# fanagislab/DBG_assembly

Hardware: AMD Instinct MI355X
Metric: M k-mers/s hashed (k=31, 150 bp) (higher is better)
Workload: dtype u64

## Files before the change

### dbg_assembly_amd/csrc/dbgk_host_level1.h

```cpp
#pragma once

#include "dbgk_l1_form.h"

constexpr L1Limits kL1Limits{(uint32_t)kL1Threads, (uint32_t)kPkWords, kPrefixMaxW, kPrefixPipeMaxB, (uint32_t)kWL1Threads, kWPkWords, kWPipePkWords};
static_assert(DBGK_L1_THREADS != 1024 || DBGK_L1_MAXB != 1024 || kL1Limits == L1Limits{}, "dbgk_l1_form.h: the defaults of L1Limits are the product build's geometry");

template <class Fn>
struct L1Row {
	L1Form form;
	Fn fn;
	uint32_t lds;
};
template <int DBG, int WIDE_D, int C, bool RAGGED, bool LIN, bool... REST>
constexpr uint32_t uniform_lds() { return LIN ? sizeof(UniformLdsLin<LIN ? C : 8>) : sizeof(UniformLds); }
#define DBGK_ROW(...) {l1_uniform(__VA_ARGS__), &k_extract_scatter_uniform<__VA_ARGS__>, uniform_lds<__VA_ARGS__>()},
static const L1Row<decltype(&k_extract_scatter_uniform<>)> kL1UniformRows[] = {DBGK_L1_UNIFORM_ROWS(DBGK_ROW)};
#undef DBGK_ROW
#define DBGK_ROW(...) {l1_prefix(__VA_ARGS__), &k_extract_scatter_prefix<__VA_ARGS__>, sizeof(PrefixLds)},
static const L1Row<decltype(&k_extract_scatter_prefix<>)> kL1PrefixRows[] = {DBGK_L1_PREFIX_ROWS(DBGK_ROW)};
#undef DBGK_ROW
#define DBGK_ROW(...) {l1_flat(__VA_ARGS__), &k_extract_scatter<__VA_ARGS__>, sizeof(ScatterLds)},
static const L1Row<decltype(&k_extract_scatter<false>)> kL1FlatRows[] = {DBGK_L1_FLAT_ROWS(DBGK_ROW)};
#undef DBGK_ROW
#define DBGK_ROW(...) {l1_flat_lin(__VA_ARGS__), &k_extract_scatter_lin<__VA_ARGS__>, sizeof(ScatterLdsLin<8>)},
static const L1Row<decltype(&k_extract_scatter_lin<false>)> kL1FlatLinRows[] = {DBGK_L1_FLAT_LIN_ROWS(DBGK_ROW)};
#undef DBGK_ROW
#define DBGK_ROW(...) {l1_wide_flat(__VA_ARGS__), &k_wide_scatter_l1<__VA_ARGS__>, sizeof(WL1Lds)},
static const L1Row<decltype(&k_wide_scatter_l1<false, 0>)> kL1WideFlatRows[] = {DBGK_L1_WIDE_FLAT_ROWS(DBGK_ROW)};
#undef DBGK_ROW
#define DBGK_ROW(WD, PIPE) {l1_wide_uniform(WD, PIPE), &k_wide_scatter_l1_uniform<WD, PIPE>, PIPE ? sizeof(WL1PipeLds) : sizeof(WL1Lds)},
static const L1Row<decltype(&k_wide_scatter_l1_uniform<0>)> kL1WideUniformRows[] = {DBGK_L1_WIDE_UNIFORM_ROWS(DBGK_ROW)};
#undef DBGK_ROW

template <class Fn, size_t N>
static int l1_set_lds_attrs(const L1Row<Fn> (&rows)[N])
{
	for (const L1Row<Fn> &r : rows)
		HIPCHK(hipFuncSetAttribute(reinterpret_cast<const void *>(r.fn), hipFuncAttributeMaxDynamicSharedMemorySize, (int)r.lds));
	return DBGK_OK;
}
static int l1_register_lds(bool wide)
{
	int rc;
	if (wide) return (rc = l1_set_lds_attrs(kL1WideFlatRows)) ? rc : l1_set_lds_attrs(kL1WideUniformRows);
	if ((rc = l1_set_lds_attrs(kL1UniformRows)) || (rc = l1_set_lds_attrs(kL1PrefixRows)) || (rc = l1_set_lds_attrs(kL1FlatRows))) return rc;
	return l1_set_lds_attrs(kL1FlatLinRows);
}

template <class Fn, size_t N, class... Args>
static int l1_launch(const L1Row<Fn> (&rows)[N], const L1Form &form, uint64_t grid, int threads, hipStream_t stream, Args... args)
{
	for (const L1Row<Fn> &r : rows)
		if (r.form == form) {
			hipLaunchKernelGGL(r.fn, dim3((uint32_t)grid), dim3(threads), r.lds, stream, args...);
			return DBGK_OK;
		}
	char text[192];
	l1_form_text(form, text, sizeof text);
	g_last_error = std::string("no level-1 kernel for the form ") + text;
	return DBGK_ERR_ARG;
}

static L1Facts l1_facts(const dbgk_handle *h, bool wrec)
{
	L1Facts f;
	f.lim = kL1Limits;
	f.part = h->part; f.seed = h->seed; f.kfreq = h->kfreq; f.wide = h->wide; f.wrec = wrec;
	f.kmer_size = h->cfg.kmer_size;
	f.max_read_len = (uint64_t)h->cfg.max_read_len;
	f.n1 = h->geom.n1; f.kf = h->geom.kf; f.geom_size = h->geom.size; f.size = h->size;
	auto hook_int = [](const char *name) { const char *v = dbgk_hook(name); return v ? atoi(v) : -1; };
	f.l1_linear = hook_int("l1_linear");
	f.l1_prefix = hook_int("l1_prefix");
	f.l1_plain = dbgk_hook("l1_plain") != nullptr;
	f.wide_l1_plain = dbgk_hook("wide_l1_plain") != nullptr;
	f.l1_flat = DBGK_EXPERIMENT_ENV("DBGK_L1_FLAT") != nullptr;
	const char *dbg = DBGK_EXPERIMENT_ENV("DBGK_DEBUG_MODE"), *lin_c = DBGK_EXPERIMENT_ENV("DBGK_L1_LINEAR_C");
	f.dbg_set = dbg != nullptr;
	f.dbg_mode = dbg ? atoi(dbg) : 0;
	f.no_reg = DBGK_EXPERIMENT_ENV("DBGK_L1_NO_REG") != nullptr;
	f.lin_c = lin_c ? (atoi(lin_c) == 12 ? 12 : 8) : 0;
	return f;
}

static int ensure_prefix_scratch(dbgk_handle *h, uint64_t n_reads, uint64_t n_bases, bool need_packed)
{
	const uint64_t tiles = (n_bases / 15 + n_reads) / kL1Threads + 2;
	if (n_reads > h->pf_cap_reads || tiles > h->pf_cap_tiles) {
		HIPCHK(hipStreamSynchronize(h->stream));
		for (void *q : {(void *)h->pf_ent, (void *)h->pf_tile_first, (void *)h->pf_tiles, (void *)h->pf_bsum})
			if (q) (void)hipFree(q);
		h->pf_ent = nullptr; h->pf_tile_first = nullptr; h->pf_tiles = nullptr; h->pf_bsum = nullptr;
		h->pf_cap_reads = h->pf_cap_tiles = 0;
		const uint64_t cr = std::max(n_reads, h->cap_reads), ct = std::max(tiles, (h->cap_bases / 15 + h->cap_reads) / kL1Threads + 2);
		const uint64_t blocks = (cr + kPrefixBlock * kPrefixItems - 1) / (kPrefixBlock * kPrefixItems) + 1;
		if (hipMalloc(&h->pf_ent, cr * sizeof(ReadLanes)) != hipSuccess || hipMalloc(&h->pf_tile_first, (ct + 1) * 4) != hipSuccess ||
		    hipMalloc(&h->pf_tiles, ct * sizeof(PrefixTile)) != hipSuccess || hipMalloc(&h->pf_bsum, blocks * 8) != hipSuccess)
			return DBGK_ERR_NOMEM;
		h->pf_cap_reads = cr;
		h->pf_cap_tiles = ct;
	}
	if (!h->pf_tot && hipMalloc(&h->pf_tot, sizeof(PrefixTotals)) != hipSuccess) return DBGK_ERR_NOMEM;
	const uint64_t words = (n_bases + 15) / 16 + 16;
	if (need_packed && words > h->pf_packed_words) {
		HIPCHK(hipStreamSynchronize(h->stream));
		if (h->pf_packed) (void)hipFree(h->pf_packed);
		h->pf_packed = nullptr;
		h->pf_packed_words = 0;
		const uint64_t cw = std::max(words, h->cap_bases / 16 + 16);
		if (hipMalloc(&h->pf_packed, cw * 4) != hipSuccess) return DBGK_ERR_NOMEM;
		h->pf_packed_words = cw;
	}
	return DBGK_OK;
}

static int early_l2(dbgk_handle *h);

template <int CC>
static void launch_prefix_passes(dbgk_handle *h, const uint64_t *d_offsets, uint64_t n_reads, uint64_t n_bases)
{
	const uint32_t n_blocks = (uint32_t)((n_reads + kPrefixBlock * kPrefixItems - 1) / (kPrefixBlock * kPrefixItems));
	const uint32_t tiles_max = (uint32_t)std::min<uint64_t>((n_bases / 15 + n_reads) / kL1Threads + 1, h->pf_cap_tiles);
	const uint32_t k = (uint32_t)h->cfg.kmer_size, max_len = (uint32_t)h->cfg.max_read_len;
	hipLaunchKernelGGL((k_prefix_count<CC>), dim3(n_blocks), dim3(kPrefixBlock), 0, h->stream, d_offsets, n_reads, k, max_len, h->pf_bsum);
	hipLaunchKernelGGL(k_prefix_blocks, dim3(1), dim3(kPrefixBlock), 0, h->stream, h->pf_bsum, n_blocks, h->pf_tot);
	hipLaunchKernelGGL((k_prefix_emit<CC>), dim3(n_blocks), dim3(kPrefixBlock), 0, h->stream, d_offsets, n_reads, k, max_len, h->pf_bsum, h->pf_ent,
	                   h->pf_tile_first, h->d_ctr);
	hipLaunchKernelGGL((k_prefix_tiles<CC>), dim3((tiles_max + 255) / 256), dim3(256), 0, h->stream, h->pf_ent, h->pf_tile_first, h->pf_tot, k, n_bases,
	                   h->pf_tiles);
}

static int launch_l1(dbgk_handle *h, const L1Plan &plan, const ReadBatch &rb, const uint64_t *d_offsets, uint64_t n_reads)
{
	for (int i = 0; i < plan.n; i++) {
		const L1Launch &l = plan.launch[i];
		const L1Geom &g = l.geom;
		const bool wide = l.form.family == L1Family::WideFlat || l.form.family == L1Family::WideUniform;
		const uint64_t wgs = (uint64_t)h->n_cu * (wide ? 1 : l1_wgs_per_cu());
		const uint64_t grid = l.tiles ? std::min(l.tiles, wgs) : wgs;
		int rc = DBGK_ERR_ARG;
		switch (l.form.family) {
		case L1Family::Uniform: {
			ReadBatch r = rb;
			if (l.n_reads != n_reads) {
				if (r.packed) r.packed += l.first_read * g.L / 16;
				else r.bases += l.first_read * g.L;
				r.n_bases = l.n_reads * g.L;
			}
			rc = l1_launch(kL1UniformRows, l.form, grid, kL1Threads, h->stream, r, UniformGeom{g.L, g.W, g.Q, g.qmagic, g.n_lanes, g.lq, g.tile_blocks},
			               d_offsets, h->geom, h->store, h->d_ctr);
			break;
		}
		case L1Family::Prefix:
			rc = l1_launch(kL1PrefixRows, l.form, grid, kL1Threads, h->stream, rb, h->pf_ent, h->pf_tiles, h->pf_tot, h->geom, h->store, h->d_ctr);
			break;
		case L1Family::Flat:
			rc = l1_launch(kL1FlatRows, l.form, grid, kL1Threads, h->stream, rb, h->geom, h->store, h->d_ctr);
			break;
		case L1Family::FlatLin:
			rc = l1_launch(kL1FlatLinRows, l.form, grid, kL1Threads, h->stream, rb, h->geom, h->store, h->d_ctr);
			break;
		case L1Family::WideFlat:
			rc = l1_launch(kL1WideFlatRows, l.form, grid, kWL1Threads, h->stream, rb, h->wgeom, h->wstore, h->wref(), h->d_ctr);
			break;
		case L1Family::WideUniform:
			rc = l1_launch(kL1WideUniformRows, l.form, grid, kWL1Threads, h->stream, rb, WUniformGeom{g.L, g.W, g.Q, g.qmagic, g.n_lanes}, h->wgeom,
			               h->wstore, h->wref(), h->d_ctr);
			break;
		}
		if (rc) return rc;
	}
	return DBGK_OK;
}

static int launch_batch(dbgk_handle *h, const char *d_bases, const uint64_t *d_offsets, uint64_t n_reads,
                        uint64_t n_bases, uint32_t *d_start, uint32_t *d_dead, int has_long ,
                        int64_t uniform_len = -1 ,
                        uint64_t len_max = 0 ,
                        const uint32_t *d_packed = nullptr )
{
	if (n_reads == 0) return DBGK_OK;
	if (h->seed && d_packed) return DBGK_ERR_ARG;
	if (h->seed) has_long = 1;
	const uint64_t words = bitmap_words(n_bases);
	TimedSpan sp;
	int rc = early_l2(h);
	if (rc) return rc;
	rc = span_begin(h, PH_MARK, sp);
	if (rc) return rc;
	static_assert(offsetof(Counters, len_max) + sizeof(unsigned long long) - offsetof(Counters, any_dead) == 20, "per-batch fields are contiguous");
	if (d_offsets) HIPCHK(hipMemsetAsync(&h->d_ctr->any_dead, 0, 20, h->stream));
	auto mark_bits = [&](int with_stats) -> int {
		HIPCHK(hipMemsetAsync(d_start, 0, words * 4, h->stream));
		if (has_long != 0) HIPCHK(hipMemsetAsync(d_dead, 0, words * 4, h->stream));
		hipLaunchKernelGGL(k_mark, dim3(grid_for(h, n_reads)), dim3(kBlock), 0, h->stream, d_offsets, n_reads, n_bases,
		                   h->cfg.kmer_size, h->cfg.max_read_len, d_start, has_long != 0 ? d_dead : nullptr, h->d_ctr, with_stats);
		return DBGK_OK;
	};
	const bool wrec = h->wide && h->wpart && !h->wbuilt;
	L1Facts facts = l1_facts(h, wrec);
	facts.n_reads = n_reads;
	facts.n_bases = n_bases;
	facts.packed = d_packed != nullptr;
	L1Plan plan{};
	int umode = -1;
	bool use_prefix = false;
	auto decide = [&]() {
		facts.has_long = has_long;
		facts.uniform_len = uniform_len;
		facts.len_max = len_max;
		plan = l1_plan(facts);
		umode = plan.umode;
		use_prefix = plan.prefix;
	};
	const bool no_offsets = d_offsets == nullptr;
	auto make_offsets = [&]() -> int {
		if (n_reads + 1 > h->uni_cap) {
			HIPCHK(hipStreamSynchronize(h->stream));
			if (h->uni_offsets) (void)hipFree(h->uni_offsets);
			h->uni_offsets = nullptr;
			h->uni_cap = 0;
			const uint64_t cap = std::max(n_reads + 1, h->cap_reads + 1);
			if (hipMalloc(&h->uni_offsets, cap * 8) != hipSuccess) return DBGK_ERR_NOMEM;
			h->uni_cap = cap;
		}
		hipLaunchKernelGGL(k_iota_offsets, dim3(grid_for(h, n_reads + 1)), dim3(kBlock), 0, h->stream, h->uni_offsets, n_reads, (uint64_t)uniform_len);
		HIPCHK(hipMemsetAsync(&h->d_ctr->any_dead, 0, 20, h->stream));
		d_offsets = h->uni_offsets;
		return DBGK_OK;
	};
	const bool may_skip_bits = (h->part && !h->seed) || wrec;
	if (may_skip_bits && has_long >= 0 && uniform_len >= 0) decide();
	if (no_offsets && umode == 1) {
		const unsigned long long w = uniform_len >= h->cfg.kmer_size ? (unsigned long long)(uniform_len - h->cfg.kmer_size + 1) * n_reads : 0ull;
		hipLaunchKernelGGL(k_add_totals, dim3(1), dim3(64), 0, h->stream, h->d_ctr, w, w);
	} else {
		if (no_offsets) {
			rc = make_offsets();
			if (rc) return rc;
		}
		if (may_skip_bits && (umode != 0 || use_prefix)) {
			hipLaunchKernelGGL(k_mark, dim3(grid_for(h, n_reads)), dim3(kBlock), 0, h->stream, d_offsets, n_reads, n_bases, h->cfg.kmer_size,
			                   h->cfg.max_read_len, (uint32_t *)nullptr, (uint32_t *)nullptr, h->d_ctr, 1);
		} else {
			rc = mark_bits(1);
			if (rc) return rc;
		}
	}
	if (h->seed && n_bases)
		hipLaunchKernelGGL(k_mark_n, dim3(grid_for(h, (n_bases + 31) >> 5)), dim3(kBlock), 0, h->stream, d_bases, n_bases, d_dead);
	HIPCHK(hipGetLastError());
	if (has_long < 0 || (uniform_len < 0 && (h->part || wrec))) {
		HIPCHK(hipMemcpyAsync(&h->h_ctr->any_dead, &h->d_ctr->any_dead, 20, hipMemcpyDeviceToHost, h->stream));
		HIPCHK(hipStreamSynchronize(h->stream));
		if (has_long < 0) has_long = h->h_ctr->any_dead ? 1 : 0;
		if (uniform_len < 0) {
			uniform_len = ~h->h_ctr->len_min_inv == h->h_ctr->len_max ? (int64_t)h->h_ctr->len_max : 0;
			len_max = h->h_ctr->len_max;
		}
	}
	if (may_skip_bits && umode < 0) {
		decide();
		if (umode == 0 && !use_prefix) {
			rc = mark_bits(0);
			if (rc) return rc;
			HIPCHK(hipGetLastError());
		}
	}
	rc = span_end(h, sp);
	if (rc) return rc;
	const uint64_t id_base = h->total_reads;
	h->total_reads += n_reads;
	if (n_bases == 0) return DBGK_OK;

	ReadBatch rb{d_bases, n_bases, d_start, has_long ? d_dead : nullptr, h->cfg.kmer_size, d_packed, &h->d_ctr->other_seen};
	const uint64_t n_chunks = (n_bases + 15) >> 4;
	rc = span_begin(h, PH_INSERT, sp);
	if (rc) return rc;
	if (h->seed) {
		hipLaunchKernelGGL(k_seed_insert, dim3(grid_for(h, n_chunks)), dim3(kBlock), 0, h->stream, rb, d_offsets, n_reads, id_base, h->tref(), h->d_ctr);
	} else if (wrec) {
		if (umode > 0) h->uniform_launches++;
		rc = launch_l1(h, plan, rb, d_offsets, n_reads);
		if (rc) return rc;
	} else if (h->wide) {
		rc = wide_ensure_zero(h);
		if (rc) return rc;
		if (has_long)
			hipLaunchKernelGGL(k_wide_extract_insert<true>, dim3(grid_for(h, n_chunks)), dim3(kBlock), 0, h->stream, rb, h->wref(), h->d_ctr);
		else
			hipLaunchKernelGGL(k_wide_extract_insert<false>, dim3(grid_for(h, n_chunks)), dim3(kBlock), 0, h->stream, rb, h->wref(), h->d_ctr);
	} else if (h->kfreq && !h->part) {
		if (has_long)
			hipLaunchKernelGGL(k_extract_count<true>, dim3(grid_for(h, n_chunks)), dim3(kBlock), 0, h->stream, rb, reinterpret_cast<uint32_t *>(h->counts));
		else
			hipLaunchKernelGGL(k_extract_count<false>, dim3(grid_for(h, n_chunks)), dim3(kBlock), 0, h->stream, rb, reinterpret_cast<uint32_t *>(h->counts));
	} else if (h->part) {
		if (use_prefix) {
			h->prefix_launches++;
			rc = ensure_prefix_scratch(h, n_reads, n_bases, d_packed == nullptr);
			if (rc) return rc;
			if (!d_packed) {
				hipLaunchKernelGGL(k_pack_bases, dim3(grid_for(h, n_chunks)), dim3(kBlock), 0, h->stream, d_bases, n_bases, h->pf_packed, h->d_ctr);
				rb.packed = h->pf_packed;
			}
			if (plan.launch[0].form.c == 15) launch_prefix_passes<15>(h, d_offsets, n_reads, n_bases);
			else launch_prefix_passes<16>(h, d_offsets, n_reads, n_bases);
		} else if (umode > 0)
			h->uniform_launches++;
		rc = launch_l1(h, plan, rb, d_offsets, n_reads);
		if (rc) return rc;
	} else if (h->track) {
		if (has_long)
			hipLaunchKernelGGL((k_extract_insert<true, true>), dim3(grid_for(h, n_chunks)), dim3(kBlock), 0, h->stream, rb, h->tref(), h->d_ctr,
			                   h->first_pos, h->pos_base);
		else
			hipLaunchKernelGGL((k_extract_insert<false, true>), dim3(grid_for(h, n_chunks)), dim3(kBlock), 0, h->stream, rb, h->tref(), h->d_ctr,
			                   h->first_pos, h->pos_base);
		h->pos_base += n_bases;
	} else if (has_long) {
		hipLaunchKernelGGL((k_extract_insert<true, false>), dim3(grid_for(h, n_chunks)), dim3(kBlock), 0, h->stream, rb, h->tref(), h->d_ctr,
		                   (unsigned long long *)nullptr, (uint64_t)0);
	} else {
		hipLaunchKernelGGL((k_extract_insert<false, false>), dim3(grid_for(h, n_chunks)), dim3(kBlock), 0, h->stream, rb, h->tref(), h->d_ctr,
		                   (unsigned long long *)nullptr, (uint64_t)0);
	}
	if (!d_packed) hipLaunchKernelGGL(k_count_other_bytes, dim3(grid_for(h, n_chunks)), dim3(kBlock), 0, h->stream, d_bases, n_bases, h->d_ctr);
	HIPCHK(hipGetLastError());
	return span_end(h, sp);
}
```

### dbg_assembly_amd/csrc/dbgk_partition.h

```cpp
#pragma once

#include <type_traits>

#include "dbgk_kernels.h"

namespace dbgk {

#ifndef DBGK_REGION_BITS
#define DBGK_REGION_BITS 12
#endif
#ifndef DBGK_BUILD_THREADS
#define DBGK_BUILD_THREADS 1024
#endif
constexpr int kRegionBits = DBGK_REGION_BITS;
constexpr int kRegionSlots = 1 << kRegionBits;
constexpr int kSpillSlots = 128;
#ifndef DBGK_L1_THREADS
#define DBGK_L1_THREADS 1024
#endif
#ifndef DBGK_L1_MAXB
#define DBGK_L1_MAXB 1024
#endif
constexpr int kTileThreads = DBGK_L1_THREADS;
constexpr int kL1MaxB = DBGK_L1_MAXB;
constexpr int kMaxBuckets = 1024;
constexpr int kSubStores = 1;
constexpr int kL1Threads = kTileThreads;
constexpr int kBuildThreads = DBGK_BUILD_THREADS;

constexpr uint64_t mod_inverse_u64(uint64_t a)
{
	uint64_t x = a;
	for (int i = 0; i < 6; i++) x *= 2 - a * x;
	return x;
}
constexpr uint64_t kInvM32 = mod_inverse_u64(1ull - (1ull << 32));
constexpr uint64_t kInvM13 = mod_inverse_u64(1ull - (1ull << 13));
constexpr uint64_t kInvM27 = mod_inverse_u64(1ull - (1ull << 27));
constexpr uint64_t kInv9 = mod_inverse_u64(9ull);

__host__ __device__ __forceinline__ uint64_t hash_code_inverse(uint64_t h)
{
	h ^= h >> 31; h ^= h >> 62;
	h = (h + 1) * kInvM27;
	h ^= h >> 15; h ^= h >> 30; h ^= h >> 60;
	h *= kInv9;
	h ^= h >> 8; h ^= h >> 16; h ^= h >> 32;
	h = (h + 1) * kInvM13;
	h ^= h >> 22; h ^= h >> 44;
	h = (h + 1) * kInvM32;
	return h;
}

struct PartGeom {
	uint64_t size;
	ModMagic magic;
	uint32_t r;
	uint32_t n1;
	uint32_t n2;
	uint32_t n_final;
	uint64_t cap1;
	uint64_t cap2;
	Div32Magic div;
	uint32_t n_ranks, rank;
	uint32_t B;
	uint32_t n_sub;
	uint32_t b_lo, nb_own;
	uint32_t n_regions_own;
	uint64_t slot_lo, slot_hi;
	uint32_t r_rec;
	uint32_t l2_shift;
	uint32_t kf;
	uint32_t kf_mask;
	uint32_t l2_records;
};

constexpr uint32_t kKfBlockBits = 16;
constexpr uint32_t kKfPermMul = 0x9E3779B1u;
constexpr uint32_t kKfPermInv = (uint32_t)mod_inverse_u64((uint64_t)kKfPermMul);

__host__ __device__ __forceinline__ uint64_t kf_slot_of_key(uint64_t key, uint32_t block_mask)
{
	const uint32_t pb = ((uint32_t)(key >> kKfBlockBits) * kKfPermMul) & block_mask;
	return ((uint64_t)pb << kKfBlockBits) | (key & ((1ull << kKfBlockBits) - 1ull));
}

__host__ __device__ __forceinline__ uint64_t kf_key_of_slot(uint64_t slot, uint32_t block_mask)
{
	const uint32_t b = ((uint32_t)(slot >> kKfBlockBits) * kKfPermInv) & block_mask;
	return ((uint64_t)b << kKfBlockBits) | (slot & ((1ull << kKfBlockBits) - 1ull));
}

struct PartStore {
	uint64_t *l1;
	uint32_t *cnt1;
	const uint64_t *inbox;
	const uint32_t *inbox_cnt;
	uint32_t *l2_done;
	uint32_t *l2_upto;
	uint64_t *l2;
	uint32_t *cnt2;
	Node *outgoing;
	unsigned long long *outgoing_n;
	uint64_t outgoing_cap;
	Node *ovf;
	Node *spill;
	unsigned long long *ovf_n;
	uint64_t ovf_cap, spill_cap;
	Node *hh;
	uint64_t hh_size;
	ModMagic hh_magic;
};

__device__ __forceinline__ uint64_t record_key(uint64_t rec, uint32_t b1, const PartGeom &G)
{
	const uint64_t v = rec >> 6;
	const uint64_t slot = ((uint64_t)b1 << G.r) | (v & ((1ull << G.r) - 1ull));
	if (G.kf == 2u) return kf_key_of_slot(slot, G.kf_mask);
	return hash_code_inverse((v >> G.r_rec) * G.size + slot);
}

__device__ __forceinline__ void push_overflow(const PartStore &P, uint64_t key, uint32_t lb, uint32_t rb, Counters *ctr)
{
	const unsigned long long i = atomicAdd(&P.ovf_n[0], 1ull);
	if (i < P.ovf_cap) {
		P.ovf[i].kmer = key;
		P.ovf[i].links = (uint64_t)lb | ((uint64_t)rb << 8);
	} else if (P.hh) {
		const TableRef T{P.hh, P.hh_size, P.hh_magic};
		const uint64_t slot = fast_mod(hash_code(key), T.magic);
		const uint4 v = *reinterpret_cast<const uint4 *>(&T.nodes[slot]);
		Node first;
		first.kmer = ((uint64_t)v.y << 32) | v.x;
		first.links = ((uint64_t)v.w << 32) | v.z;
		uint64_t guess;
		unsigned long long dummy_new = 0, dummy_conf = 0;
		const uint64_t s = find_or_claim(T, key, slot, first, guess, dummy_new, dummy_conf);
		if (s == ~0ull)
			atomicOr(&ctr->error, 2u);
		else
			links_cas_observe(reinterpret_cast<unsigned long long *>(&T.nodes[s].links), guess, lb, rb);
	} else {
		atomicOr(&ctr->error, 2u);
	}
}

__device__ __forceinline__ void lds_barrier()
{
	asm volatile("s_waitcnt lgkmcnt(0)\n\ts_barrier" ::: "memory");
}

__device__ __forceinline__ uint32_t fresh_tid()
{
	uint32_t t = threadIdx.x;
	asm volatile("" : "+v"(t));
	return t;
}

template <int THREADS, int MAXB = kMaxBuckets, bool FLAT_DESC = false>
struct ScatterLdsT {
	static constexpr int kThreads = THREADS;
	static constexpr int kRecords = THREADS * 16;
	static constexpr int kMaxB = MAXB;
	static constexpr int kBpt = MAXB / THREADS;
	using Desc = typename std::conditional<FLAT_DESC, uint32_t, uint64_t>::type;
	uint64_t stage[kRecords];
	uint32_t hist[MAXB + 64];
	uint32_t lbase[MAXB];
	Desc desc[MAXB];
	uint32_t wave_tot[THREADS / 64];
};
using ScatterLds = ScatterLdsT<kTileThreads, kL1MaxB>;
#ifndef DBGK_L2_THREADS
#define DBGK_L2_THREADS 512
#endif
constexpr int l2_threads(int maxb) { return maxb <= 1024 ? 2 * DBGK_L2_THREADS : DBGK_L2_THREADS; }
template <int MAXB> using ScatterLdsL2T = ScatterLdsT<l2_threads(MAXB), MAXB, true>;
using ScatterLdsL2 = ScatterLdsL2T<kMaxBuckets>;
constexpr int kMaxBucketsL2 = 4096;

template <class LDS>
__device__ __forceinline__ uint32_t scan_hist(LDS &L)
{
	const int t = (int)fresh_tid(), lane = t & 63, wave = t >> 6;
	constexpr int kBpt = LDS::kBpt;
	uint32_t v[kBpt], sum = 0;
#pragma unroll
	for (int j = 0; j < LDS::kBpt; j++) { v[j] = L.hist[LDS::kBpt * t + j]; sum += v[j]; }
	uint32_t inc = sum;
#pragma unroll
	for (int off = 1; off < 64; off <<= 1) {
		const uint32_t n = __shfl_up(inc, off, 64);
		if (lane >= off) inc += n;
	}
	if (lane == 63) L.wave_tot[wave] = inc;
	lds_barrier();
	uint32_t run = inc - sum, all = 0;
#pragma unroll
	for (int w = 0; w < LDS::kThreads / 64; w++) {
		const uint32_t wt = L.wave_tot[w];
		run += (w < wave) ? wt : 0u;
		all += wt;
	}
#pragma unroll
	for (int j = 0; j < LDS::kBpt; j++) { L.lbase[LDS::kBpt * t + j] = run; run += v[j]; }
	return all;
}

template <class LDS>
__device__ __forceinline__ void scan_hist_per_wave(LDS &L, uint32_t n_buckets, uint32_t hist_off = 0u)
{
	const uint32_t *hist = L.hist + hist_off;
	const uint32_t lane = fresh_tid() & 63u;
	const uint32_t E = (n_buckets + 63u) >> 6;
	uint32_t sum = 0;
	for (uint32_t j = 0; j < E; j++) {
		const uint32_t b = E * lane + j;
		sum += b < (uint32_t)LDS::kMaxB ? hist[b] : 0u;
	}
	uint32_t inc = sum;
#pragma unroll
	for (int off = 1; off < 64; off <<= 1) {
		const uint32_t n = __shfl_up(inc, off, 64);
		if ((int)lane >= off) inc += n;
	}
	uint32_t run = inc - sum;
	for (uint32_t j = 0; j < E; j++) {
		const uint32_t b = E * lane + j;
		if (b < (uint32_t)LDS::kMaxB) {
			const uint32_t c = hist[b];
			L.lbase[b] = run;
			run += c;
		}
	}
}

__device__ __forceinline__ uint32_t wave_scan_inclusive_dpp(uint32_t v)
{
	v += (uint32_t)__builtin_amdgcn_update_dpp(0, (int)v, 0x111, 0xf, 0xf, false);
	v += (uint32_t)__builtin_amdgcn_update_dpp(0, (int)v, 0x112, 0xf, 0xf, false);
	v += (uint32_t)__builtin_amdgcn_update_dpp(0, (int)v, 0x114, 0xf, 0xf, false);
	v += (uint32_t)__builtin_amdgcn_update_dpp(0, (int)v, 0x118, 0xf, 0xf, false);
	v += (uint32_t)__builtin_amdgcn_update_dpp(0, (int)v, 0x142, 0xa, 0xf, false);
	v += (uint32_t)__builtin_amdgcn_update_dpp(0, (int)v, 0x143, 0xc, 0xf, false);
	return v;
}

constexpr uint32_t kScanStraightB = 256;
template <class LDS>
__device__ __forceinline__ void scan_hist_per_wave_256(LDS &L, uint32_t hist_off = 0u)
{
	static_assert(LDS::kMaxB >= (int)kScanStraightB && offsetof(LDS, hist) % 16 == 0 && offsetof(LDS, lbase) % 16 == 0, "16-byte LDS accesses of whole entries");
	const uint32_t lane = fresh_tid() & 63u;
	const uint4 v = *reinterpret_cast<const uint4 *>(L.hist + hist_off + 4u * lane);
	const uint32_t sum = (v.x + v.y) + (v.z + v.w);
	const uint32_t run = wave_scan_inclusive_dpp(sum) - sum;
	*reinterpret_cast<uint4 *>(L.lbase + 4u * lane) = make_uint4(run, run + v.x, run + v.x + v.y, run + v.x + v.y + v.z);
}


template <class LDS>
__device__ __forceinline__ uint32_t scatter_reserve_scan(LDS &L, uint32_t n_buckets, uint32_t *__restrict__ cnt, uint32_t (&my_gbase)[LDS::kBpt],
                                                         uint32_t stride = 1u)
{
	const int t = (int)fresh_tid();
#pragma unroll
	for (int j = 0; j < LDS::kBpt; j++) {
		const uint32_t b = LDS::kBpt * t + j, c = L.hist[b];
		my_gbase[j] = (b < n_buckets && c) ? atomicAdd(&cnt[b * stride], c) : 0u;
	}
	const uint32_t all = scan_hist(L);
	lds_barrier();
	return all;
}

template <int PER_THREAD, int DBG = 0, bool FLAT = false, bool KF32_POSSIBLE = true, int N_SURE = 0, class LDS>
__device__ __forceinline__ void scatter_stage_copy(LDS &L, const uint64_t (&rec)[PER_THREAD], const uint32_t (&br)[PER_THREAD],
                                                   const uint32_t (&my_gbase)[LDS::kBpt], uint32_t n_buckets, uint64_t *__restrict__ out,
                                                   uint64_t cap, uint32_t b1_of_bucket0, bool bucket_is_b1, const PartGeom &G,
                                                   const PartStore &P, Counters *ctr, uint32_t stride = 1u,
                                                   uint32_t flat_total = 0u,
                                                   bool sure = false)
{
	const int t = (int)fresh_tid();
	if (FLAT) {
#pragma unroll
		for (int j = 0; j < LDS::kBpt; j++) L.hist[LDS::kBpt * t + j] = 0;
	}
	bool staged = false;
	if constexpr (N_SURE > 0) {
		if (__builtin_amdgcn_ballot_w64(!sure) == 0ull) {
			uint32_t at[N_SURE];
#pragma unroll
			for (int u = 0; u < N_SURE; u++) at[u] = L.lbase[br[u] >> 16];
#pragma unroll
			for (int u = 0; u < N_SURE; u++) L.stage[at[u] + (br[u] & 0xFFFFu)] = rec[u];
			staged = true;
		}
	}
	if (!staged) {
#pragma unroll
		for (int u = 0; u < PER_THREAD; u++) {
			if ((br[u] >> 16) < (uint32_t)LDS::kMaxB) L.stage[L.lbase[br[u] >> 16] + (br[u] & 0xFFFFu)] = rec[u];
			if ((u & 3) == 3) __builtin_amdgcn_sched_barrier(0);
		}
	}
#pragma unroll
	for (int j = 0; j < LDS::kBpt; j++) {
		const uint32_t b = LDS::kBpt * t + j;
		if (FLAT) L.desc[b] = (typename LDS::Desc)(my_gbase[j] - L.lbase[b]);
		else L.desc[b] = (typename LDS::Desc)(((uint64_t)my_gbase[j] << 32) | (L.hist[b] << 16) | L.lbase[b]);
	}
	lds_barrier();
	if (FLAT) {
		if (DBG != 2) {
			const uint32_t total = flat_total;
#pragma unroll
			for (int u = 0; u < PER_THREAD; u++) {
				const uint32_t p = (uint32_t)u * LDS::kThreads + (uint32_t)t;
				if (p >= total) continue;
				const uint64_t rcd = L.stage[p];
				const uint32_t b = (uint32_t)(rcd >> (6 + kRegionBits + G.l2_shift)) & (n_buckets - 1u);
				const uint64_t off = (uint32_t)((uint32_t)L.desc[b] + p);
				if (DBG == 3) {
					out[(uint64_t)blockIdx.x * 4096u + (((uint64_t)b * cap + off) & 4095ull)] = rcd;
				} else if (off < cap) {
					if (G.kf == 2u) reinterpret_cast<uint16_t *>(out)[(uint64_t)b * cap + off] = (uint16_t)(rcd >> 6);
					else out[(uint64_t)b * cap + off] = rcd;
				} else {
					const uint32_t b1 = bucket_is_b1 ? b : b1_of_bucket0;
					push_overflow(P, record_key(rcd, b1, G), (uint32_t)(rcd >> 3) & 7u, (uint32_t)rcd & 7u, ctr);
				}
			}
		}
		return;
	}
	const uint32_t lane = t & 63, wave = __builtin_amdgcn_readfirstlane((uint32_t)t >> 6);
	constexpr uint32_t kWaves = LDS::kThreads / 64;
	const uint32_t per_wave = (DBG == 2) ? 0u : (n_buckets + kWaves - 1u - wave) / kWaves;
	const uint32_t mine = wave + kWaves * lane;
	const uint64_t d = (lane < per_wave) ? (uint64_t)L.desc[mine] : 0ull;
	const uint32_t d_lo = (uint32_t)d, d_hi = (uint32_t)(d >> 32);
	for (uint32_t kk = 0; kk < per_wave; kk++) {
		const uint32_t k = __builtin_amdgcn_readfirstlane(kk);
		const uint32_t lo = __builtin_amdgcn_readlane(d_lo, k), dst = __builtin_amdgcn_readlane(d_hi, k);
		const uint32_t n = lo >> 16, src = lo & 0xFFFFu;
		if (n == 0) continue;
		const uint32_t b = wave + kWaves * k;
		if (KF32_POSSIBLE && G.kf == 2u) {
			static_assert(kSubStores == 1, "the 32-bit level-1 store is addressed without sub-stores");
			uint32_t *o32 = reinterpret_cast<uint32_t *>(out) + (uint64_t)b * cap + dst;
			if ((uint64_t)dst + n <= cap) {
				typedef uint32_t u32x4_a4 __attribute__((ext_vector_type(4), aligned(4)));
				if (n >= 4u) {
					for (uint32_t i = 4u * lane; i < n; i += 256u) {
						const uint32_t j = min(i, n - 4u);
						const u32x4_a4 v = {(uint32_t)L.stage[src + j], (uint32_t)L.stage[src + j + 1u], (uint32_t)L.stage[src + j + 2u], (uint32_t)L.stage[src + j + 3u]};
						*reinterpret_cast<u32x4_a4 *>(o32 + j) = v;
					}
				} else if (lane < n) {
					o32[lane] = (uint32_t)L.stage[src + lane];
				}
			} else {
				for (uint32_t i = lane; i < n; i += 64) {
					const uint64_t rcd = L.stage[src + i];
					if ((uint64_t)dst + i < cap) o32[i] = (uint32_t)rcd;
					else push_overflow(P, record_key(rcd, bucket_is_b1 ? b : b1_of_bucket0, G), (uint32_t)(rcd >> 3) & 7u, (uint32_t)rcd & 7u, ctr);
				}
			}
			continue;
		}
		uint64_t *o = out + (uint64_t)b * stride * cap + dst;
		if (DBG == 3) {
			for (uint32_t i = lane; i < n; i += 64) out[(uint64_t)blockIdx.x * 4096u + (((uint64_t)b * stride * cap + dst + i) & 4095ull)] = L.stage[src + i];
		} else if ((uint64_t)dst + n <= cap) {
			typedef uint32_t u32x4_a8 __attribute__((ext_vector_type(4), aligned(8)));
			if (n >= 2u) {
				for (uint32_t i = 2u * lane; i < n; i += 128u) {
					const uint32_t j = min(i, n - 2u);
					const uint64_t a = L.stage[src + j], b2 = L.stage[src + j + 1u];
					const u32x4_a8 v = {(uint32_t)a, (uint32_t)(a >> 32), (uint32_t)b2, (uint32_t)(b2 >> 32)};
					*reinterpret_cast<u32x4_a8 *>(o + j) = v;
				}
			} else if (lane == 0u) {
				o[0] = L.stage[src];
			}
		} else {
			for (uint32_t i = lane; i < n; i += 64) {
				const uint64_t rcd = L.stage[src + i];
				if ((uint64_t)dst + i < cap) {
					o[i] = rcd;
				} else {
					const uint32_t b1 = bucket_is_b1 ? b : b1_of_bucket0;
					push_overflow(P, record_key(rcd, b1, G), (uint32_t)(rcd >> 3) & 7u, (uint32_t)rcd & 7u, ctr);
				}
			}
		}
	}
}

template <int PER_THREAD, int DBG = 0, bool FLAT = false, class LDS>
__device__ __forceinline__ void scatter_tile(LDS &L, const uint64_t (&rec)[PER_THREAD], uint32_t (&bkt)[PER_THREAD],
                                             uint32_t n_buckets, uint32_t *__restrict__ cnt, uint64_t *__restrict__ out,
                                             uint64_t cap, uint32_t b1_of_bucket0, bool bucket_is_b1, const PartGeom &G,
                                             const PartStore &P, Counters *ctr)
{
#pragma unroll
	for (int u = 0; u < PER_THREAD; u++) bkt[u] = (bkt[u] << 16) | ((bkt[u] != 0xFFFFu) ? atomicAdd(&L.hist[bkt[u]], 1u) : 0u);
	lds_barrier();
	if (DBG == 1) {
		uint64_t x = 0;
#pragma unroll
		for (int u = 0; u < PER_THREAD; u++) x ^= rec[u] + bkt[u];
		if (x == 0x1234567u) out[threadIdx.x] = x;
		return;
	}
	uint32_t my_gbase[LDS::kBpt];
	const uint32_t all = scatter_reserve_scan(L, n_buckets, cnt, my_gbase);
	static_assert(FLAT, "scatter_tile is level 2's: the flat copy-out clears the histogram for the next tile");
	scatter_stage_copy<PER_THREAD, DBG, FLAT, false>(L, rec, bkt, my_gbase, n_buckets, out, cap, b1_of_bucket0, bucket_is_b1, G, P, ctr, 1u, all);
}


__device__ __forceinline__ uint64_t sliding_or(uint64_t x, uint32_t w)
{
	uint64_t res = 0ull, cur = x;
	uint32_t done = 0;
#pragma unroll
	for (uint32_t j = 0; j < 6; j++) {
		if (w & (1u << j)) {
			res |= cur >> done;
			done += 1u << j;
		}
		cur |= cur >> (1u << j);
	}
	return res;
}

struct Chunk16 {
	uint64_t kbit, rc;
	uint32_t nb;
	uint32_t lw;
	uint32_t valid, has_l, has_r;
};

__device__ __forceinline__ uint4 load_ascii16(const char *__restrict__ bases, uint64_t n_bases, uint64_t chunk)
{
	const uint64_t off = chunk * 16u;
	if (off + 16u <= n_bases) return *reinterpret_cast<const uint4 *>(bases + off);
	uint32_t w[4] = {0x41414141u, 0x41414141u, 0x41414141u, 0x41414141u};
	for (uint64_t i = 0; off + i < n_bases && i < 16; i++) {
		const uint32_t c = (uint8_t)bases[off + i];
		w[i >> 2] = (w[i >> 2] & ~(0xFFu << ((i & 3u) * 8u))) | (c << ((i & 3u) * 8u));
	}
	return make_uint4(w[0], w[1], w[2], w[3]);
}

struct RawChunk {
	uint4 a0;
	uint4 halo;
	uint32_t prevb;
	uint32_t s0, s1, s2, d0, d1, d2;
};

template <bool HAS_DEAD, bool GUARDED>
__device__ __forceinline__ RawChunk load_raw(const ReadBatch &rb, uint64_t chunk, uint64_t n_chunks)
{
	RawChunk r;
	const uint32_t lane = fresh_tid() & 63u;
	const uint64_t halo_chunk = chunk - lane + 64u + lane;
	r.a0 = make_uint4(0x41414141u, 0x41414141u, 0x41414141u, 0x41414141u);
	r.halo = r.a0;
	r.prevb = 0x41u;
	if (rb.packed) {
		r.a0.x = r.halo.x = r.prevb = 0u;
		if (GUARDED) {
			if (chunk < n_chunks) r.a0.x = packed_word(rb, chunk);
			if (lane < 2u && halo_chunk < n_chunks) r.halo.x = packed_word(rb, halo_chunk);
		} else {
			r.a0.x = rb.packed[chunk];
			if (lane < 2u) r.halo.x = rb.packed[halo_chunk];
		}
		if (lane == 0u && chunk > 0u && (!GUARDED || chunk * 16u - 1u < rb.n_bases)) r.prevb = rb.packed[chunk - 1u] & 3u;
	} else if (GUARDED) {
		if (chunk < n_chunks) r.a0 = load_ascii16(rb.bases, rb.n_bases, chunk);
		if (lane < 2u && halo_chunk < n_chunks) r.halo = load_ascii16(rb.bases, rb.n_bases, halo_chunk);
	} else {
		r.a0 = *reinterpret_cast<const uint4 *>(rb.bases + chunk * 16u);
		if (lane < 2u) r.halo = *reinterpret_cast<const uint4 *>(rb.bases + halo_chunk * 16u);
	}
	if (!rb.packed && lane == 0u && chunk > 0u && (!GUARDED || chunk * 16u - 1u < rb.n_bases)) r.prevb = (uint8_t)rb.bases[chunk * 16u - 1u];
	const uint64_t p0 = chunk * 16u;
	const uint64_t wi = p0 >> 5;
	r.s0 = r.s1 = r.s2 = r.d0 = r.d1 = r.d2 = 0u;
	if (!GUARDED || chunk < n_chunks) {
		r.s0 = rb.start_bits[wi];
		r.s1 = rb.start_bits[wi + 1];
		r.s2 = rb.start_bits[wi + 2];
		if (HAS_DEAD) {
			r.d0 = rb.dead_bits[wi];
			r.d1 = rb.dead_bits[wi + 1];
			r.d2 = rb.dead_bits[wi + 2];
		}
	}
	return r;
}

__device__ __forceinline__ uint64_t bits64_from_words(uint32_t w0, uint32_t w1, uint32_t w2, uint32_t sh)
{
	const uint64_t lo = (uint64_t)w0 | ((uint64_t)w1 << 32);
	return sh ? (lo >> sh) | ((uint64_t)w2 << (64u - sh)) : lo;
}

template <bool HAS_DEAD>
__device__ __forceinline__ Chunk16 decode_chunk16(const RawChunk &raw, const ReadBatch &rb, uint64_t chunk)
{
	Chunk16 c;
	const uint32_t k = (uint32_t)rb.k;
	const uint32_t lane = fresh_tid() & 63u;
	const uint64_t p0 = chunk * 16u;
	const uint4 h0 = make_uint4(__builtin_amdgcn_readlane(raw.halo.x, 0), __builtin_amdgcn_readlane(raw.halo.y, 0),
	                            __builtin_amdgcn_readlane(raw.halo.z, 0), __builtin_amdgcn_readlane(raw.halo.w, 0));
	const uint4 h1 = make_uint4(__builtin_amdgcn_readlane(raw.halo.x, 1), __builtin_amdgcn_readlane(raw.halo.y, 1),
	                            __builtin_amdgcn_readlane(raw.halo.z, 1), __builtin_amdgcn_readlane(raw.halo.w, 1));
	uint32_t w0, hw0, hw1, pb;
	if (rb.packed) {
		w0 = raw.a0.x; hw0 = h0.x; hw1 = h1.x;
		pb = __builtin_amdgcn_readlane(raw.prevb, 0);
	} else {
		w0 = pack16_ascii(raw.a0, rb.other_seen);
		hw0 = pack16_ascii(h0, rb.other_seen); hw1 = pack16_ascii(h1, rb.other_seen);
		pb = code_ascii(__builtin_amdgcn_readlane(raw.prevb, 0), rb.other_seen);
	}
	uint32_t w1 = __shfl_down(w0, 1, 64), w2 = __shfl_down(w0, 2, 64);
	if (lane == 63u) { w1 = hw0; w2 = hw1; }
	if (lane == 62u) w2 = hw0;
	uint32_t prev = __shfl_up(w0, 1, 64) & 3u;
	if (lane == 0u) prev = pb;
	if (chunk == 0u) prev = 0u;
	const uint64_t S = bits64_from_words(raw.s0, raw.s1, raw.s2, (uint32_t)(p0 & 31u));
	const uint64_t hi = ((uint64_t)w0 << 32) | w1, mid = ((uint64_t)w1 << 32) | w2;
	const uint32_t sh = 64u - 2u * k;
	c.kbit = hi >> sh;
	c.rc = revcomp_kbit(c.kbit, (int)k);
	c.nb = (sh < 32u) ? (uint32_t)(mid >> sh) : (uint32_t)(hi >> (sh - 32u));
	c.lw = (prev << 30) | (w0 >> 2);
	uint64_t bad = sliding_or(S >> 1, k - 1u);
	uint64_t no_r = S >> k;
	if (HAS_DEAD) {
		const uint64_t D = bits64_from_words(raw.d0, raw.d1, raw.d2, (uint32_t)(p0 & 31u));
		bad |= sliding_or(D, k);
		no_r |= D >> k;
	}
	const uint64_t room = rb.n_bases > p0 ? rb.n_bases - p0 : 0ull;
	const uint32_t nv = room >= k ? (uint32_t)(room - k + 1u < 16u ? room - k + 1u : 16u) : 0u;
	const uint32_t nr = room > k ? (uint32_t)(room - k < 16u ? room - k : 16u) : 0u;
	c.valid = ~(uint32_t)bad & ((1u << nv) - 1u);
	c.has_r = ~(uint32_t)no_r & ((1u << nr) - 1u);
	c.has_l = ~(uint32_t)S & 0xFFFFu & (p0 ? 0xFFFFu : 0xFFFEu);
	return c;
}

}

#include "dbgk_partition_l1.h"
#include "dbgk_partition_l2.h"
#include "dbgk_partition_build.h"

namespace dbgk {

__global__ __launch_bounds__(kBlock) void k_insert_triples(const Node *__restrict__ in, const unsigned long long *__restrict__ n_ptr,
                                                           uint64_t cap, TableRef T, Counters *__restrict__ ctr)
{
	__shared__ unsigned long long red[kBlock / 64];
	unsigned long long n_new = 0, n_conf = 0;
	bool full = false;
	const uint64_t n = *n_ptr < cap ? *n_ptr : cap;
	const uint64_t stride = (uint64_t)gridDim.x * kBlock;
	for (uint64_t i = (uint64_t)blockIdx.x * kBlock + threadIdx.x; i < n; i += stride) {
		const uint64_t key = in[i].kmer;
		const uint32_t lb = (uint32_t)in[i].links & 0xFFu, rb = (uint32_t)(in[i].links >> 8) & 0xFFu;
		uint64_t slot = fast_mod(hash_code(key), T.magic);
		const uint4 f = *reinterpret_cast<const uint4 *>(&T.nodes[slot]);
		Node first;
		first.kmer = ((uint64_t)f.y << 32) | f.x;
		first.links = ((uint64_t)f.w << 32) | f.z;
		uint64_t guess;
		const uint64_t s = find_or_claim(T, key, slot, first, guess, n_new, n_conf);
		if (s == ~0ull) { full = true; continue; }
		links_cas_observe(reinterpret_cast<unsigned long long *>(&T.nodes[s].links), guess, lb, rb);
	}
	const unsigned long long a = block_sum(n_new, red);
	const unsigned long long b = block_sum(n_conf, red);
	if (threadIdx.x == 0) {
		if (a) atomicAdd(&ctr->n_new, a);
		if (b) atomicAdd(&ctr->n_conflict, b);
	}
	if (full) atomicOr(&ctr->error, 1u);
}

__global__ __launch_bounds__(kBlock) void k_merge_spill(const Node *__restrict__ in, const unsigned long long *__restrict__ n_ptr,
                                                        uint64_t cap, TableRef T, Counters *__restrict__ ctr)
{
	__shared__ unsigned long long red[kBlock / 64];
	unsigned long long n_new = 0, n_conf = 0;
	bool full = false;
	const uint64_t n = *n_ptr < cap ? *n_ptr : cap;
	const uint64_t stride = (uint64_t)gridDim.x * kBlock;
	for (uint64_t i = (uint64_t)blockIdx.x * kBlock + threadIdx.x; i < n; i += stride) {
		const uint64_t key = in[i].kmer, add = in[i].links;
		uint64_t slot = fast_mod(hash_code(key), T.magic);
		const uint4 f = *reinterpret_cast<const uint4 *>(&T.nodes[slot]);
		Node first;
		first.kmer = ((uint64_t)f.y << 32) | f.x;
		first.links = ((uint64_t)f.w << 32) | f.z;
		uint64_t guess;
		const uint64_t s = find_or_claim(T, key, slot, first, guess, n_new, n_conf);
		if (s == ~0ull) { full = true; continue; }
		links_cas_merge(reinterpret_cast<unsigned long long *>(&T.nodes[s].links), guess, add);
	}
	const unsigned long long a = block_sum(n_new, red);
	const unsigned long long b = block_sum(n_conf, red);
	if (threadIdx.x == 0) {
		if (a) atomicAdd(&ctr->n_new, a);
		if (b) atomicAdd(&ctr->n_conflict, b);
	}
	if (full) atomicOr(&ctr->error, 1u);
}

__device__ __forceinline__ uint64_t find_or_claim_range(Node *nodes, uint64_t slot_lo, uint64_t slot_hi, uint64_t key, uint64_t slot,
                                                        uint64_t &links_guess, unsigned long long &n_new, unsigned long long &n_conf)
{
	for (; slot < slot_hi; slot++) {
		const uint64_t idx = slot - slot_lo;
		const uint4 v = *reinterpret_cast<const uint4 *>(&nodes[idx]);
		uint64_t seen = ((uint64_t)v.y << 32) | v.x;
		uint64_t links = ((uint64_t)v.w << 32) | v.z;
		if (seen == 0ull) {
			seen = atomicCAS(reinterpret_cast<unsigned long long *>(&nodes[idx].kmer), 0ull, (unsigned long long)key);
			if (seen == 0ull) {
				n_new++;
				links_guess = 0ull;
				return idx;
			}
			links = 0ull;
		}
		if (seen == key) {
			links_guess = links;
			return idx;
		}
		n_conf++;
	}
	return ~0ull;
}

__global__ __launch_bounds__(kBlock) void k_merge_sharded(const Node *__restrict__ in, const unsigned long long *__restrict__ n_ptr,
                                                          uint64_t n_direct, uint64_t cap, int is_triple, int start_foreign_at_lo,
                                                          PartGeom G, PartStore P, Node *__restrict__ table, Counters *__restrict__ ctr)
{
	__shared__ unsigned long long red[kBlock / 64];
	unsigned long long n_new = 0, n_conf = 0;
	uint64_t n = n_ptr ? (uint64_t)*n_ptr : n_direct;
	if (n > cap) n = cap;
	const uint64_t stride = (uint64_t)gridDim.x * kBlock;
	for (uint64_t i = (uint64_t)blockIdx.x * kBlock + threadIdx.x; i < n; i += stride) {
		const uint64_t key = in[i].kmer;
		uint64_t add = in[i].links;
		if (is_triple) add = links_observe(0ull, (uint32_t)add & 0xFFu, (uint32_t)(add >> 8) & 0xFFu);
		if (key == 0ull) {
			if (add) links_cas_merge(&ctr->polyA_links, 0ull, add);
			continue;
		}
		const uint64_t home = fast_mod(hash_code(key), G.magic);
		const bool mine = home >= G.slot_lo && home < G.slot_hi;
		if (!mine && !start_foreign_at_lo) continue;
		uint64_t guess;
		const uint64_t idx = find_or_claim_range(table, G.slot_lo, G.slot_hi, key, mine ? home : G.slot_lo, guess, n_new, n_conf);
		if (idx == ~0ull) {
			const unsigned long long j = atomicAdd(P.outgoing_n, 1ull);
			if (j < P.outgoing_cap) {
				P.outgoing[j].kmer = key;
				P.outgoing[j].links = add;
			} else {
				atomicOr(&ctr->error, 2u);
			}
			continue;
		}
		links_cas_merge(reinterpret_cast<unsigned long long *>(&table[idx].links), guess, add);
	}
	const unsigned long long a = block_sum(n_new, red);
	const unsigned long long b = block_sum(n_conf, red);
	if (threadIdx.x == 0) {
		if (a) atomicAdd(&ctr->n_new, a);
		if (b) atomicAdd(&ctr->n_conflict, b);
	}
}

}
```

### dbg_assembly_amd/csrc/dbgk_partition_l1.h

```cpp
#pragma once

namespace dbgk {

struct NoMid { __device__ __forceinline__ void operator()(uint32_t) const {} };
template <int WIDE_D, int NPOS = 16, class LDS = ScatterLds, bool SPECIAL = false, bool ROLL32 = SPECIAL, bool IN_REGS = false, bool ZERO_POSSIBLE = true,
          class Mid = NoMid>
__device__ __forceinline__ bool l1_positions(LDS &L, const PartGeom &G, Chunk16 c, uint32_t tid, uint64_t head_mask, uint32_t rc_shift,
                                             uint32_t rel_mask, uint32_t q_shift, uint32_t (&bkt)[16], uint64_t *rec = nullptr,
                                             uint32_t hist_off = 0u, Mid mid = Mid())
{
	static_assert(!IN_REGS || SPECIAL || ROLL32 || WIDE_D == 3, "records in registers: regular tiles of a graph handle, or a KFREQ handle with direct blocks (nothing to patch)");
	static_assert(ZERO_POSSIBLE || ((SPECIAL || ROLL32) && WIDE_D != 3), "the positions without the zero-key test: the 32-bit-roll forms of a graph handle");
	uint32_t *const hh = L.hist + (IN_REGS ? hist_off : 0u);
	const uint32_t lwc = ~c.lw, nbc = ~c.nb;
	uint32_t rev_mask = 0;
	bool zero_any = false;
	uint32_t zero_acc = 0u;
#pragma unroll
	for (uint32_t i = NPOS; i < 16; i++) bkt[i] = (uint32_t)kL1MaxB << 16;
#pragma unroll
	for (uint32_t i = 0; i < (uint32_t)NPOS; i++) {
		mid(i);
		const uint32_t sh = 30u - 2u * i;
		const uint32_t left = (c.lw >> sh) & 3u, right = (c.nb >> sh) & 3u;
		const bool rev = c.rc < c.kbit;
		const uint64_t key = rev ? c.rc : c.kbit;
		uint32_t links = 4u;
		if constexpr (WIDE_D == 3) {
		} else if constexpr (ROLL32) {
			uint32_t wa = rev ? nbc : c.lw, wb = rev ? lwc : c.nb;
			asm volatile("" : "+v"(wa), "+v"(wb));
			links = (((wa >> sh) & 3u) << 3) | ((wb >> sh) & 3u);
			if constexpr (!SPECIAL) links = G.kf ? 4u : links;
		} else {
			uint32_t lf = (left << 3) | right, lr = (((nbc >> sh) & 3u) << 3) | ((lwc >> sh) & 3u);
			asm volatile("" : "+v"(lf), "+v"(lr));
			links = G.kf ? 4u : (rev ? lr : lf);
		}
		if (WIDE_D != 3 && (!SPECIAL || i == 0u || i == (uint32_t)NPOS - 1u)) {
			uint32_t rev_bit = rev ? 1u : 0u;
			asm volatile("" : "+v"(rev_bit));
			rev_mask = SPECIAL ? (rev_mask | (rev_bit << ((uint32_t)NPOS - 1u - i))) : ((rev_mask << 1) | rev_bit);
		}
		uint64_t q;
		uint32_t slot, bucket;
		if constexpr (WIDE_D == 3) {
			const uint64_t s64 = kf_slot_of_key(key, G.kf_mask);
			q = 0ull;
			slot = (uint32_t)s64;
			bucket = (uint32_t)(s64 >> G.r);
		} else if (WIDE_D == 2) {
			uint64_t s64;
			if (G.kf == 2u) {
				s64 = kf_slot_of_key(key, G.kf_mask);
				q = 0ull;
			} else {
				s64 = fast_divmod(hash_code(key), G.magic, q);
			}
			slot = (uint32_t)s64;
			bucket = (uint32_t)(s64 >> G.r);
		} else {
			slot = WIDE_D ? divmod_u64_u32(hash_code(key), G.div, q) : divmod_magic_small(hash_code(key), G.magic.m, (uint32_t)G.magic.d, q);
			bucket = slot >> G.r;
		}
		const uint32_t q_lo = (uint32_t)q, q_hi = (uint32_t)(q >> 32);
		const uint32_t rec_lo = (((q_lo << (q_shift - 6u)) | (slot & rel_mask)) << 6) | links;
		const uint32_t rec_hi = __builtin_amdgcn_alignbit(q_hi, q_lo, 32u - q_shift);
		if constexpr (IN_REGS) {
			uint32_t lo_now = rec_lo, hi_now = rec_hi;
			if constexpr (WIDE_D == 3) {
				asm volatile("" : "+v"(lo_now));
				rec[i] = lo_now;
			} else {
				asm volatile("" : "+v"(lo_now), "+v"(hi_now));
				rec[i] = ((uint64_t)hi_now << 32) | lo_now;
			}
			if (i > 0u) asm volatile("" : "+v"(bkt[i - 1u]));
		} else {
			L.stage[i * kL1Threads + tid] = ((uint64_t)rec_hi << 32) | rec_lo;
		}
		const bool valid = SPECIAL ? true : (bool)((c.valid >> i) & 1u);
		const bool zero = ZERO_POSSIBLE ? key == 0ull : false;
		if constexpr (!ZERO_POSSIBLE) {
		} else if constexpr (IN_REGS) {
			zero_acc = zero ? 1u : zero_acc;
			asm volatile("" : "+v"(zero_acc));
		} else {
			zero_any = zero_any || zero;
		}
		const uint32_t b = (valid && !zero) ? bucket : (uint32_t)kL1MaxB + (tid & 63u);
		bkt[i] = (b << 16) | atomicAdd(&hh[b], 1u);
		if constexpr (ROLL32) {
			const uint32_t klo = (uint32_t)c.kbit, khi = (uint32_t)(c.kbit >> 32);
			const uint32_t nhi = __builtin_amdgcn_alignbit(khi, klo, 30u) & (uint32_t)(head_mask >> 32), nlo = (klo << 2) | right;
			c.kbit = ((uint64_t)nhi << 32) | nlo;
			const uint64_t r2 = c.rc >> 2;
			c.rc = ((uint64_t)((uint32_t)(r2 >> 32) | ((right ^ 3u) << (rc_shift - 32u))) << 32) | (uint32_t)r2;
		} else {
			c.kbit = ((c.kbit << 2) | right) & head_mask;
			c.rc = (c.rc >> 2) | ((uint64_t)(3u - right) << rc_shift);
		}
	}
	const uint32_t no_l = ~c.has_l & 0xFFFFu, no_r = ~c.has_r & 0xFFFFu;
	if constexpr (IN_REGS && !SPECIAL && WIDE_D != 3) {
		if (const uint32_t fix = G.kf ? 0u : (no_l | no_r) & c.valid) {
#pragma unroll
			for (uint32_t i = 0; i < (uint32_t)NPOS; i++) {
				if (!((fix >> i) & 1u)) continue;
				const bool nl = (no_l >> i) & 1u, nr = (no_r >> i) & 1u;
				const bool fwd = !((rev_mask >> ((uint32_t)NPOS - 1u - i)) & 1u);
				uint32_t lb = ((uint32_t)rec[i] >> 3) & 7u, rbb = (uint32_t)rec[i] & 7u;
				if (fwd ? nl : nr) lb = 4u;
				if (fwd ? nr : nl) rbb = 4u;
				rec[i] = (rec[i] & ~63ull) | (lb << 3) | rbb;
			}
		}
		return zero_acc != 0u;
	} else if constexpr (IN_REGS) {
#pragma unroll
		for (uint32_t e = 0; e < (WIDE_D == 3 ? 0u : 2u); e++) {
			const uint32_t i = e ? (uint32_t)NPOS - 1u : 0u;
			if (e && NPOS == 1) break;
			const bool nl = (no_l >> i) & 1u, nr = (no_r >> i) & 1u;
			if (nl || nr) {
				const bool fwd = !((rev_mask >> ((uint32_t)NPOS - 1u - i)) & 1u);
				uint32_t lb = ((uint32_t)rec[i] >> 3) & 7u, rbb = (uint32_t)rec[i] & 7u;
				if (fwd ? nl : nr) lb = 4u;
				if (fwd ? nr : nl) rbb = 4u;
				rec[i] = (rec[i] & ~63ull) | (lb << 3) | rbb;
			}
		}
		return zero_acc != 0u;
	}
	for (uint32_t fix = (WIDE_D == 3 || (!SPECIAL && G.kf)) ? 0u : ((no_l | no_r) & c.valid); fix; fix &= fix - 1u) {
		const uint32_t i = (uint32_t)__builtin_ctz(fix);
		const bool fwd = !((rev_mask >> ((uint32_t)NPOS - 1u - i)) & 1u), nl = (no_l >> i) & 1u, nr = (no_r >> i) & 1u;
		uint64_t rec = L.stage[i * kL1Threads + tid];
		uint32_t lb = ((uint32_t)rec >> 3) & 7u, rbb = (uint32_t)rec & 7u;
		if (fwd ? nl : nr) lb = 4u;
		if (fwd ? nr : nl) rbb = 4u;
		L.stage[i * kL1Threads + tid] = (rec & ~63ull) | (lb << 3) | rbb;
	}
	return zero_any;
}

template <int DBG, bool KF32_POSSIBLE = true, int N_SURE = 0>
__device__ __forceinline__ void l1_scatter_tail(ScatterLds &L, const PartGeom &G, const PartStore &P, Counters *ctr, uint32_t tid,
                                                const uint32_t (&bkt)[16], bool sure = false)
{
	lds_barrier();
	uint64_t rec[16];
#pragma unroll
	for (int u = 0; u < 16; u++) rec[u] = (N_SURE == 0 || u < N_SURE) ? L.stage[u * kL1Threads + tid] : 0ull;
	uint32_t my_gbase[ScatterLds::kBpt];
	const uint32_t sub = blockIdx.x % G.n_sub;
	scatter_reserve_scan(L, G.n1, P.cnt1 + sub, my_gbase, G.n_sub);
	scatter_stage_copy<16, DBG, false, KF32_POSSIBLE, N_SURE>(L, rec, bkt, my_gbase, G.n1, P.l1 + (uint64_t)sub * G.cap1, G.cap1, 0u, true, G, P, ctr, G.n_sub, 0u, sure);
}

template <int C>
struct ScatterLdsLin {
	static constexpr int kThreads = kL1Threads;
	static constexpr int kRecords = kL1Threads * C;
	static constexpr int kMaxB = kL1MaxB;
	static constexpr int kBpt = kL1MaxB / kL1Threads;
	using Desc = uint32_t;
	uint64_t stage[kRecords];
	uint32_t hist[kL1MaxB + 64];
	uint32_t lbase[kL1MaxB];
	uint32_t desc[kL1MaxB];
	uint32_t wave_tot[kL1Threads / 64];
	uint16_t bucket_of[kRecords];
};

template <int DBG, int C, bool KF32_POSSIBLE = true>
__device__ __forceinline__ void l1_scatter_tail_linear(ScatterLdsLin<C> &L, const PartGeom &G, const PartStore &P, Counters *ctr, uint32_t tid,
                                                       const uint32_t (&bkt)[16])
{
	using ScatterLds8 = ScatterLdsLin<C>;
	lds_barrier();
	uint64_t rec[C];
#pragma unroll
	for (int u = 0; u < C; u++) rec[u] = L.stage[u * kL1Threads + tid];
	uint32_t my_gbase[ScatterLds8::kBpt];
	const uint32_t sub = blockIdx.x % G.n_sub;
	scatter_reserve_scan(L, G.n1, P.cnt1 + sub, my_gbase, G.n_sub);
	const uint32_t total = L.lbase[G.n1 - 1u] + L.hist[G.n1 - 1u];
#pragma unroll
	for (int u = 0; u < C; u++) {
		const uint32_t b = bkt[u] >> 16;
		if (b < (uint32_t)kL1MaxB) {
			const uint32_t at = L.lbase[b] + (bkt[u] & 0xFFFFu);
			L.stage[at] = rec[u];
			L.bucket_of[at] = (uint16_t)b;
		}
	}
#pragma unroll
	for (int j = 0; j < ScatterLds8::kBpt; j++) L.desc[ScatterLds8::kBpt * tid + j] = my_gbase[j];
	lds_barrier();
	if (DBG != 2) {
		uint64_t *out = P.l1 + (uint64_t)sub * G.cap1;
#pragma unroll
		for (int u = 0; u < C; u++) {
			const uint32_t p = (uint32_t)u * kL1Threads + fresh_tid();
			if (p >= total) continue;
			const uint64_t rcd = L.stage[p];
			const uint32_t b = L.bucket_of[p];
			const uint64_t off = (uint64_t)L.desc[b] + (p - L.lbase[b]);
			if (off < G.cap1) {
				if (KF32_POSSIBLE && G.kf == 2u) reinterpret_cast<uint32_t *>(out)[(uint64_t)b * G.cap1 + off] = (uint32_t)rcd;
				else out[(uint64_t)b * G.n_sub * G.cap1 + off] = rcd;
			} else {
				push_overflow(P, record_key(rcd, b, G), (uint32_t)(rcd >> 3) & 7u, (uint32_t)rcd & 7u, ctr);
			}
		}
	}
}

template <bool HAS_DEAD, int DBG = 0, int WIDE_D = 0>
__global__ __launch_bounds__(kL1Threads) void k_extract_scatter(ReadBatch rb, PartGeom G, PartStore P, Counters *__restrict__ ctr)
{
	extern __shared__ __align__(16) unsigned char lds_raw[];
	ScatterLds &L = *reinterpret_cast<ScatterLds *>(lds_raw);
	const uint64_t n_chunks = (rb.n_bases + 15u) >> 4;
	const uint64_t n_tiles = (n_chunks + kL1Threads - 1) / kL1Threads;
	const uint32_t k = (uint32_t)rb.k;
	const uint64_t head_mask = (k < 32u) ? ((1ull << (2u * k)) - 1ull) : ~0ull;
	const uint32_t rc_shift = 2u * k - 2u;
	const uint32_t rel_mask = (1u << G.r) - 1u, q_shift = G.r + 6u;

	auto interior = [&](uint64_t tile) { return ((tile + 1u) * kL1Threads + 2u) * 16u <= rb.n_bases; };
	auto fetch = [&](uint64_t tile) {
		const uint64_t ch = tile * kL1Threads + fresh_tid();
		if (tile >= n_tiles) return RawChunk{};
		return interior(tile) ? load_raw<HAS_DEAD, false>(rb, ch, n_chunks) : load_raw<HAS_DEAD, true>(rb, ch, n_chunks);
	};
	RawChunk raw = fetch(blockIdx.x);
	for (uint64_t tile = blockIdx.x; tile < n_tiles; tile += gridDim.x) {
		const uint32_t tid = fresh_tid();
		const uint64_t chunk = tile * kL1Threads + tid;
		uint32_t bkt[16];
#pragma unroll
		for (int j = 0; j < ScatterLds::kBpt; j++) L.hist[ScatterLds::kBpt * tid + j] = 0;
		lds_barrier();
		Chunk16 c = decode_chunk16<HAS_DEAD>(raw, rb, chunk);
		if (chunk >= n_chunks) c.valid = 0u;
		const bool zero_seen = l1_positions<WIDE_D>(L, G, c, tid, head_mask, rc_shift, rel_mask, q_shift, bkt);
		if (zero_seen && chunk < n_chunks) {
			LaneWindow w = load_lane_window<HAS_DEAD>(rb, chunk);
#pragma unroll 1
			for (uint32_t i = 0; i < 16; i++) {
				const Triple tr = next_triple<HAS_DEAD>(w, i, rb.k, rb.n_bases);
				if (tr.valid && tr.key == 0ull)
					links_cas_observe(&ctr->polyA_links, *reinterpret_cast<volatile unsigned long long *>(&ctr->polyA_links),
					                  G.kf ? 0u : tr.lb, G.kf ? 4u : tr.rb);
			}
		}
		if (DBG == 1) {
			uint64_t x = 0;
#pragma unroll
			for (int u = 0; u < 16; u++) x ^= L.stage[u * kL1Threads + tid] + bkt[u];
			if (x == 0x1234567u) P.l1[threadIdx.x] = x;
			lds_barrier();
			raw = fetch(tile + gridDim.x);
			continue;
		}
		const RawChunk nxt = fetch(tile + gridDim.x);
		l1_scatter_tail<DBG, (WIDE_D >= 2)>(L, G, P, ctr, tid, bkt);
		raw = nxt;
	}
}

template <bool HAS_DEAD, int WIDE_D = 0>
__global__ __launch_bounds__(kL1Threads) void k_extract_scatter_lin(ReadBatch rb, PartGeom G, PartStore P, Counters *__restrict__ ctr)
{
	extern __shared__ __align__(16) unsigned char lds_raw[];
	using LDS = ScatterLdsLin<8>;
	LDS &L = *reinterpret_cast<LDS *>(lds_raw);
	const uint64_t n_chunks = (rb.n_bases + 15u) >> 4;
	const uint64_t n_tiles = (n_chunks + kL1Threads - 1) / kL1Threads;
	const uint32_t k = (uint32_t)rb.k;
	const uint64_t head_mask = (k < 32u) ? ((1ull << (2u * k)) - 1ull) : ~0ull;
	const uint32_t rc_shift = 2u * k - 2u;
	const uint32_t rel_mask = (1u << G.r) - 1u, q_shift = G.r + 6u;
	auto interior = [&](uint64_t tile) { return ((tile + 1u) * kL1Threads + 2u) * 16u <= rb.n_bases; };
	auto fetch = [&](uint64_t tile) {
		const uint64_t ch = tile * kL1Threads + fresh_tid();
		if (tile >= n_tiles) return RawChunk{};
		return interior(tile) ? load_raw<HAS_DEAD, false>(rb, ch, n_chunks) : load_raw<HAS_DEAD, true>(rb, ch, n_chunks);
	};
	RawChunk raw = fetch(blockIdx.x);
	for (uint64_t tile = blockIdx.x; tile < n_tiles; tile += gridDim.x) {
		const uint64_t chunk = tile * kL1Threads + fresh_tid();
		Chunk16 c = decode_chunk16<HAS_DEAD>(raw, rb, chunk);
		if (chunk >= n_chunks) c.valid = 0u;
		raw = fetch(tile + gridDim.x);
		bool zero_any = false;
#pragma unroll 1
		for (uint32_t half = 0; half < 2u; half++) {
			const uint32_t tid = fresh_tid();
			uint32_t bkt[16];
#pragma unroll
			for (int j = 0; j < LDS::kBpt; j++) L.hist[LDS::kBpt * tid + j] = 0;
			lds_barrier();
			Chunk16 h8 = c;
			h8.valid &= 0xFFu;
			h8.has_l = (h8.has_l & 0xFFu) | 0xFF00u;
			h8.has_r = (h8.has_r & 0xFFu) | 0xFF00u;
			zero_any = l1_positions<WIDE_D, 8, LDS>(L, G, h8, tid, head_mask, rc_shift, rel_mask, q_shift, bkt) || zero_any;
			c.kbit = ((c.kbit << 16) | (uint64_t)(c.nb >> 16)) & head_mask;
			c.rc = revcomp_kbit(c.kbit, (int)k);
			c.lw <<= 16;
			c.nb <<= 16;
			c.valid >>= 8;
			c.has_l >>= 8;
			c.has_r >>= 8;
			l1_scatter_tail_linear<0, 8, (WIDE_D >= 2)>(L, G, P, ctr, tid, bkt);
		}
		if (zero_any && chunk < n_chunks) {
			LaneWindow w = load_lane_window<HAS_DEAD>(rb, chunk);
#pragma unroll 1
			for (uint32_t i = 0; i < 16; i++) {
				const Triple tr = next_triple<HAS_DEAD>(w, i, rb.k, rb.n_bases);
				if (tr.valid && tr.key == 0ull)
					links_cas_observe(&ctr->polyA_links, *reinterpret_cast<volatile unsigned long long *>(&ctr->polyA_links),
					                  G.kf ? 0u : tr.lb, G.kf ? 4u : tr.rb);
			}
		}
	}
}

struct UniformGeom {
	uint32_t L;
	uint32_t W;
	uint32_t Q;
	uint32_t qmagic;
	uint64_t n_lanes;
	uint32_t lq;
	uint32_t tile_blocks;
};

constexpr int kPkWords = 1792 * kTileThreads / 1024;
struct UniformLds {
	ScatterLds s;
	uint32_t pk[kPkWords];
	uint32_t gbase[kL1MaxB];
};
template <int C>
struct UniformLdsLin {
	ScatterLdsLin<C> s;
	uint32_t pk[kPkWords];
};

__device__ __forceinline__ uint32_t funnel_left(uint32_t hi, uint32_t lo, uint32_t sh)
{
	uint32_t f = __builtin_amdgcn_alignbit(hi, lo, 32u - sh);
	asm volatile("" : "+v"(f));
	return sh ? f : hi;
}

__device__ __forceinline__ uint32_t l1_word_runs(uint32_t x0, uint32_t x1, uint32_t x2, uint32_t x3, uint32_t x4)
{
	return min(min(min(x0 + 1u, x1 + 1u), min(x2 + 1u, x3 + 1u)), x4 + 1u);
}
__device__ __forceinline__ bool l1_no_zero_key(uint32_t k, uint32_t word_runs)
{
	return k >= 31u && __builtin_amdgcn_ballot_w64(word_runs < 2u) == 0ull;
}

__device__ __forceinline__ void l1_key0_from_chunk(Chunk16 c, uint64_t head_mask, uint32_t rc_shift, uint32_t kf, Counters *ctr)
{
#pragma unroll 1
	for (uint32_t i = 0; i < 16; i++) {
		const uint32_t sh = 30u - 2u * i;
		const uint32_t left = (c.lw >> sh) & 3u, right = (c.nb >> sh) & 3u;
		const bool rev = c.rc < c.kbit;
		const uint64_t key = rev ? c.rc : c.kbit;
		if (((c.valid >> i) & 1u) && key == 0ull) {
			const uint32_t lc = ((c.has_l >> i) & 1u) ? left : 4u, rcd = ((c.has_r >> i) & 1u) ? right : 4u;
			const uint32_t lb = rev ? (rcd == 4u ? 4u : 3u - rcd) : lc, rb = rev ? (lc == 4u ? 4u : 3u - lc) : rcd;
			links_cas_observe(&ctr->polyA_links, *reinterpret_cast<volatile unsigned long long *>(&ctr->polyA_links), kf ? 0u : lb, kf ? 4u : rb);
		}
		c.kbit = ((c.kbit << 2) | right) & head_mask;
		c.rc = (c.rc >> 2) | ((uint64_t)(3u - right) << rc_shift);
	}
}

template <bool REC32>
struct L1Pipe {
	static constexpr uint32_t kWaves = kL1Threads / 64;
	static constexpr uint32_t kHist2 = (uint32_t)((offsetof(ScatterLds, desc) - offsetof(ScatterLds, hist)) / 4u);
	static_assert(sizeof(ScatterLds::desc) >= sizeof(ScatterLds::hist), "the second histogram lives in the descriptor array");
	static_assert(kL1MaxB <= kL1Threads, "thread b reserves bucket b");
	static_assert(kHist2 % 4u == 0u, "scan_hist_per_wave_256 reads either histogram sixteen bytes at a time");
	ScatterLds &L;
	uint32_t *const gbase;
	const PartGeom &G;
	const PartStore &P;
	Counters *const ctr;
	uint32_t tid, lane, wave, per_wave, mine;
	uint64_t *out;
	uint32_t *cnt;
	uint64_t bucket_stride;
	uint32_t d_lo = 0u, d_gb = 0u;
	uint32_t cur = 0u;

	__device__ __forceinline__ L1Pipe(ScatterLds &L_, uint32_t *gbase_, const PartGeom &G_, const PartStore &P_, Counters *ctr_)
	    : L(L_), gbase(gbase_), G(G_), P(P_), ctr(ctr_)
	{
		tid = fresh_tid();
		lane = tid & 63u;
		wave = __builtin_amdgcn_readfirstlane(tid >> 6);
		per_wave = (G.n1 + kWaves - 1u - wave) / kWaves;
		mine = wave + kWaves * lane;
		const uint32_t sub = blockIdx.x % G.n_sub;
		out = P.l1 + (uint64_t)sub * G.cap1;
		cnt = P.cnt1 + sub;
		bucket_stride = (uint64_t)G.n_sub * G.cap1;
	}
	__device__ __forceinline__ uint32_t *stage32() const { return reinterpret_cast<uint32_t *>(L.stage); }

	__device__ __forceinline__ void copy_run(uint32_t kk, uint64_t &slow) const
	{
		const uint32_t lo = __builtin_amdgcn_readlane(d_lo, kk), dst = __builtin_amdgcn_readlane(d_gb, kk);
		const uint32_t n = lo >> 16, src = lo & 0xFFFFu;
		if (n == 0u) return;
		if ((uint64_t)dst + n > G.cap1) {
			slow |= 1ull << kk;
			return;
		}
		uint32_t b = wave + kWaves * kk;
		asm volatile("" : "+s"(b));
		if constexpr (REC32) {
			static_assert(kSubStores == 1, "the 32-bit level-1 store is addressed without sub-stores");
			uint32_t *o32 = reinterpret_cast<uint32_t *>(out) + (uint64_t)b * G.cap1 + dst;
			const uint32_t *s32 = stage32();
			typedef uint32_t u32x4_a4 __attribute__((ext_vector_type(4), aligned(4)));
			if (n >= 4u) {
				for (uint32_t i = 4u * lane; i < n; i += 256u) {
					const uint32_t j = min(i, n - 4u);
					const u32x4_a4 v = {s32[src + j], s32[src + j + 1u], s32[src + j + 2u], s32[src + j + 3u]};
					*reinterpret_cast<u32x4_a4 *>(o32 + j) = v;
				}
			} else if (lane < n) {
				o32[lane] = s32[src + lane];
			}
			return;
		}
		uint64_t *o = out + (uint64_t)b * bucket_stride + dst;
		typedef uint32_t u32x4_a8 __attribute__((ext_vector_type(4), aligned(8)));
		if (n >= 2u) {
			for (uint32_t i = 2u * lane; i < n; i += 128u) {
				const uint32_t j = min(i, n - 2u);
				const uint64_t a = L.stage[src + j], b2 = L.stage[src + j + 1u];
				const u32x4_a8 v = {(uint32_t)a, (uint32_t)(a >> 32), (uint32_t)b2, (uint32_t)(b2 >> 32)};
				*reinterpret_cast<u32x4_a8 *>(o + j) = v;
			}
		} else if (lane == 0u) {
			o[0] = L.stage[src];
		}
	}
	__device__ __forceinline__ void copy_slow(uint64_t slow) const
	{
		while (slow) {
			const uint32_t kk = __builtin_amdgcn_readfirstlane((uint32_t)__builtin_ctzll(slow));
			slow &= slow - 1ull;
			const uint32_t lo = __builtin_amdgcn_readlane(d_lo, kk), dst = __builtin_amdgcn_readlane(d_gb, kk);
			const uint32_t n = lo >> 16, src = lo & 0xFFFFu, b = wave + kWaves * kk;
			uint64_t *o = out + (uint64_t)b * G.n_sub * G.cap1 + dst;
			uint32_t *o32 = reinterpret_cast<uint32_t *>(out) + (uint64_t)b * G.cap1 + dst;
			for (uint32_t i = lane; i < n; i += 64u) {
				const uint64_t rcd = REC32 ? (uint64_t)stage32()[src + i] : L.stage[src + i];
				if ((uint64_t)dst + i < G.cap1) {
					if constexpr (REC32) o32[i] = (uint32_t)rcd;
					else o[i] = rcd;
				} else push_overflow(P, record_key(rcd, b, G), (uint32_t)(rcd >> 3) & 7u, (uint32_t)rcd & 7u, ctr);
			}
		}
	}
	__device__ __forceinline__ void copy_rest(uint32_t from, uint64_t slow) const
	{
		for (uint32_t kk = from; kk < per_wave; kk++) copy_run(__builtin_amdgcn_readfirstlane(kk), slow);
		if (slow) copy_slow(slow);
	}
	template <int C, bool SURE, class Open>
	__device__ __forceinline__ void tail(const uint64_t (&rec)[16], const uint32_t (&bkt)[16], bool zero_seen, Open open_next)
	{
		const uint32_t c_t = tid < G.n1 ? L.hist[cur + tid] : 0u;
		const uint32_t g_t = c_t ? atomicAdd(&cnt[tid * G.n_sub], c_t) : 0u;
		const uint32_t c_mine = lane < per_wave ? L.hist[cur + mine] : 0u;
		if (G.n1 <= kScanStraightB) scan_hist_per_wave_256(L, cur);
		else scan_hist_per_wave(L, G.n1, cur);
		d_lo = (c_mine << 16) | (lane < per_wave ? L.lbase[mine] : 0u);
		if (SURE && __builtin_amdgcn_ballot_w64(zero_seen) == 0ull) {
			uint32_t at[C];
#pragma unroll
			for (int u = 0; u < C; u++) at[u] = L.lbase[bkt[u] >> 16];
#pragma unroll
			for (int u = 0; u < C; u++) L.stage[at[u] + (bkt[u] & 0xFFFFu)] = rec[u];
		} else {
#pragma unroll
			for (int u = 0; u < C; u++)
				if ((bkt[u] >> 16) < (uint32_t)kL1MaxB) {
					if constexpr (REC32) stage32()[L.lbase[bkt[u] >> 16] + (bkt[u] & 0xFFFFu)] = (uint32_t)rec[u];
					else L.stage[L.lbase[bkt[u] >> 16] + (bkt[u] & 0xFFFFu)] = rec[u];
				}
		}
		if (tid < G.n1) gbase[tid] = g_t;
		open_next(cur ^ kHist2);
		lds_barrier();
		d_gb = lane < per_wave ? gbase[mine] : 0u;
		cur ^= kHist2;
	}
};

template <int DBG = 0, int WIDE_D = 0, int C = 16, bool RAGGED = false, bool LIN = false, bool REG = false, bool PACKED = false, bool FULL = true,
          bool K17 = REG>
__global__ __launch_bounds__(kL1Threads) void k_extract_scatter_uniform(ReadBatch rb, UniformGeom U, const uint64_t *__restrict__ offsets,
                                                                         PartGeom G, PartStore P, Counters *__restrict__ ctr)
{
	static_assert(!LIN || C == 8 || C == 12, "the linear form stages 8 or 12 records per thread");
	static_assert(!REG || (!RAGGED && !LIN), "regular tiles: equal-length reads, wave-per-bucket form");
	static_assert(!PACKED || REG, "the other forms test rb.packed at run time");
	static_assert(FULL || (REG && DBG == 0), "partly filled lanes: the pipelined regular tiles");
	static_assert(K17 || !REG, "regular tiles: k >= 17");
	using ULds = typename std::conditional<LIN, UniformLdsLin<LIN ? C : 8>, UniformLds>::type;
	using SLds = typename std::conditional<LIN, ScatterLdsLin<LIN ? C : 8>, ScatterLds>::type;
	extern __shared__ __align__(16) unsigned char lds_raw[];
	ULds &UL = *reinterpret_cast<ULds *>(lds_raw);
	SLds &L = UL.s;
	const uint64_t n_tiles = (U.n_lanes + kL1Threads - 1) / kL1Threads;
	const uint32_t k = (uint32_t)rb.k;
	const uint64_t head_mask = (k < 32u) ? ((1ull << (2u * k)) - 1ull) : ~0ull;
	const uint32_t rc_shift = 2u * k - 2u;
	const uint32_t rel_mask = (1u << G.r) - 1u, q_shift = G.r + 6u;

	const uint64_t stride_lanes = (uint64_t)gridDim.x * kL1Threads;
	const uint64_t stride_r = stride_lanes / U.Q;
	const uint32_t stride_c = (uint32_t)(stride_lanes - stride_r * U.Q);
	uint64_t r0 = ((uint64_t)blockIdx.x * kL1Threads) / U.Q;
	uint32_t c0 = (uint32_t)((uint64_t)blockIdx.x * kL1Threads - r0 * U.Q);

	auto read_start = [&](uint64_t r) -> uint64_t { return RAGGED ? offsets[r] : r * U.L; };
	using Block = typename std::conditional<PACKED, uint32_t, uint4>::type;
	struct RawU {
		Block a, b;
		uint64_t B0;
		uint64_t p;
		uint32_t n_blocks;
		uint32_t cc;
		uint32_t W;
	};
	auto fetch = [&](uint64_t tile, uint64_t rr, uint32_t c_first) {
		RawU raw;
		if constexpr (PACKED) raw.a = raw.b = 0u;
		else raw.a = raw.b = make_uint4(0x41414141u, 0x41414141u, 0x41414141u, 0x41414141u);
		raw.B0 = raw.p = 0;
		raw.n_blocks = raw.cc = raw.W = 0;
		if (tile >= n_tiles) return raw;
		const uint32_t t = fresh_tid();
		if constexpr (REG) {
			raw.B0 = tile * ((uint64_t)U.tile_blocks * 16u);
			raw.n_blocks = U.tile_blocks;
			if constexpr (PACKED) {
				const uint32_t *words = rb.packed + (raw.B0 >> 4);
				if (t < raw.n_blocks) raw.a = words[t];
				if (t + kL1Threads < raw.n_blocks) raw.b = words[t + kL1Threads];
			} else {
				const uint4 *blocks = reinterpret_cast<const uint4 *>(rb.bases + raw.B0);
				if (t < raw.n_blocks) raw.a = blocks[t];
				if (t + kL1Threads < raw.n_blocks) raw.b = blocks[t + kL1Threads];
			}
			raw.cc = t & (U.Q - 1u);
			raw.p = raw.B0 + (t >> U.lq) * U.L + (uint32_t)C * raw.cc;
			raw.W = U.W;
			return raw;
		}
		const uint64_t p_first = RAGGED ? min(offsets[rr] + (uint32_t)C * c_first, offsets[rr + 1]) : read_start(rr) + (uint32_t)C * c_first;
		raw.B0 = (p_first ? p_first - 1u : 0u) & ~15ull;
		const uint64_t lane_last = min((tile + 1u) * kL1Threads, U.n_lanes) - 1u;
		const uint32_t xl = c_first + (uint32_t)(lane_last - tile * kL1Threads);
		const uint32_t drl = (xl * U.qmagic) >> 22;
		uint64_t end = read_start(rr + drl) + (uint32_t)C * (xl - drl * U.Q) + (uint32_t)C + k + 2u;
		end = min(end, (rb.n_bases + 15u) & ~15ull);
		raw.n_blocks = end > raw.B0 ? min((uint32_t)((end - raw.B0 + 15u) >> 4), (uint32_t)kPkWords) : 0u;
		if constexpr (!PACKED) {
			if (rb.packed) {
				if (t < raw.n_blocks) raw.a.x = packed_word(rb, (raw.B0 >> 4) + t);
				if (t + kL1Threads < raw.n_blocks) raw.b.x = packed_word(rb, (raw.B0 >> 4) + t + kL1Threads);
			} else {
				if (t < raw.n_blocks) raw.a = load_ascii16(rb.bases, rb.n_bases, (raw.B0 >> 4) + t);
				if (t + kL1Threads < raw.n_blocks) raw.b = load_ascii16(rb.bases, rb.n_bases, (raw.B0 >> 4) + t + kL1Threads);
			}
		}
		const uint32_t x = c_first + t;
		const uint32_t dr = (x * U.qmagic) >> 22;
		raw.cc = x - dr * U.Q;
		if (tile * kL1Threads + t < U.n_lanes) {
			const uint64_t r = rr + dr;
			const uint64_t s = read_start(r);
			const uint64_t len = RAGGED ? offsets[r + 1] - s : (uint64_t)U.L;
			raw.p = s + (uint32_t)C * raw.cc;
			raw.W = len >= k ? (uint32_t)(len - k + 1u) : 0u;
		}
		return raw;
	};

	RawU raw = fetch(blockIdx.x, r0, c0);
	auto open_tile = [&](const RawU &rw, uint32_t hist_off = 0u) {
		const uint32_t tid = fresh_tid();
		if constexpr (PACKED) {
			if (tid < rw.n_blocks) UL.pk[tid] = rw.a;
			if (tid + kL1Threads < rw.n_blocks) UL.pk[tid + kL1Threads] = rw.b;
		} else if (rb.packed) {
			if (tid < rw.n_blocks) UL.pk[tid] = rw.a.x;
			if (tid + kL1Threads < rw.n_blocks) UL.pk[tid + kL1Threads] = rw.b.x;
		} else {
			if (tid < rw.n_blocks) UL.pk[tid] = pack16_ascii(rw.a, rb.other_seen);
			if (tid + kL1Threads < rw.n_blocks) UL.pk[tid + kL1Threads] = pack16_ascii(rw.b, rb.other_seen);
		}
#pragma unroll
		for (int j = 0; j < SLds::kBpt; j++) L.hist[hist_off + SLds::kBpt * tid + j] = 0;
	};
	auto decode = [&](const RawU &raw, uint32_t *word_runs = nullptr) {
		if constexpr (REG && FULL) {
			const uint32_t t = fresh_tid();
			const uint32_t cc = t & (U.Q - 1u);
			const bool first = cc == 0u, last = cc == U.Q - 1u;
			const uint32_t rel = (t >> U.lq) * U.L + (uint32_t)C * cc - (first ? 0u : 1u);
			const uint32_t d = rel >> 4, sh = 2u * (rel & 15u);
			const uint32_t x0 = UL.pk[d], x1 = UL.pk[d + 1], x2 = UL.pk[d + 2], x3 = UL.pk[d + 3], x4 = UL.pk[d + 4];
			if (word_runs) *word_runs = l1_word_runs(x0, x1, x2, x3, x4);
			const uint32_t X0 = funnel_left(x0, x1, sh), X1 = funnel_left(x1, x2, sh), X2 = funnel_left(x2, x3, sh), X3 = funnel_left(x3, x4, sh);
			const uint32_t adv = first ? 0u : 2u;
			const uint32_t Y0 = funnel_left(X0, X1, adv), Y1 = funnel_left(X1, X2, adv), Y2 = funnel_left(X2, X3, adv), Y3 = X3 << adv;
			Chunk16 c;
			c.lw = first ? (X0 >> 2) : X0;
			c.kbit = ((((uint64_t)Y0 << 32) | Y1)) >> (64u - 2u * k);
			c.rc = revcomp_kbit(c.kbit, (int)k);
			const bool k32 = (k >> 4) == 2u;
			const uint32_t wsh = 2u * (k & 15u);
			c.nb = funnel_left(k32 ? Y2 : Y1, k32 ? Y3 : Y2, wsh);
			c.valid = (1u << C) - 1u;
			c.has_r = last ? (1u << (C - 1)) - 1u : (1u << C) - 1u;
			c.has_l = first ? 0xFFFEu : 0xFFFFu;
			return c;
		}
		const uint64_t p = raw.p;
		const bool no_prev = REG ? raw.cc == 0u : p == 0u;
		const uint64_t s0 = no_prev ? p : p - 1u;
		const uint32_t first_w = (uint32_t)C * raw.cc;
		const bool live = first_w < raw.W;
		Chunk16 c;
		const uint32_t rel = live ? (uint32_t)(s0 - raw.B0) : 0u;
		const uint32_t d = min(rel >> 4, (uint32_t)kPkWords - 5u), sh = 2u * (rel & 15u);
		const uint32_t x0 = UL.pk[d], x1 = UL.pk[d + 1], x2 = UL.pk[d + 2], x3 = UL.pk[d + 3], x4 = UL.pk[d + 4];
		if (word_runs) *word_runs = l1_word_runs(x0, x1, x2, x3, x4);
		const uint32_t X0 = funnel_left(x0, x1, sh), X1 = funnel_left(x1, x2, sh), X2 = funnel_left(x2, x3, sh), X3 = funnel_left(x3, x4, sh);
		const uint32_t adv = no_prev ? 0u : 2u;
		const uint32_t Y0 = funnel_left(X0, X1, adv), Y1 = funnel_left(X1, X2, adv), Y2 = funnel_left(X2, X3, adv), Y3 = X3 << adv;
		c.lw = no_prev ? (X0 >> 2) : X0;
		c.kbit = ((((uint64_t)Y0 << 32) | Y1)) >> (64u - 2u * k);
		c.rc = revcomp_kbit(c.kbit, (int)k);
		const uint32_t widx = k >> 4, wsh = 2u * (k & 15u);
		const uint32_t ya = widx == 0u ? Y0 : (widx == 1u ? Y1 : Y2), yb = widx == 0u ? Y1 : (widx == 1u ? Y2 : Y3);
		c.nb = funnel_left(ya, yb, wsh);
		const uint32_t nv = live ? min((uint32_t)C, raw.W - first_w) : 0u;
		const uint32_t nr = (live && first_w + 1u < raw.W) ? min((uint32_t)C, raw.W - 1u - first_w) : 0u;
		c.valid = (1u << nv) - 1u;
		c.has_r = (1u << nr) - 1u;
		c.has_l = raw.cc ? 0xFFFFu : 0xFFFEu;
		return c;
	};
	constexpr bool kRec32 = WIDE_D == 3;
	constexpr bool kPipe = !LIN && DBG == 0 && (REG || K17 || (kRec32 && !RAGGED));
	constexpr bool kZeroPerWave = K17 && !kRec32;
	if constexpr (kPipe) {
		L1Pipe<kRec32> pp(L, UL.gbase, G, P, ctr);
		const uint32_t tid = pp.tid;
		if (blockIdx.x < n_tiles) {
			open_tile(raw, 0u);
			lds_barrier();
		}
		for (uint64_t tile = blockIdx.x; tile < n_tiles; tile += gridDim.x) {
			uint32_t word_runs = 0u;
			const Chunk16 c = decode(raw, &word_runs);
			uint32_t bkt[16];
			uint64_t rec[16];
			uint64_t slow = 0ull;
			auto mid = [&](uint32_t i) { pp.copy_run(i, slow); };
			bool zero_seen;
			if constexpr (kZeroPerWave) {
				if (l1_no_zero_key(k, word_runs))
					zero_seen = l1_positions<WIDE_D, C, SLds, REG && FULL, K17, true, false>(L, G, c, tid, head_mask, rc_shift, rel_mask, q_shift, bkt, rec, pp.cur, mid);
				else
					zero_seen = l1_positions<WIDE_D, C, SLds, REG && FULL, K17, true, true>(L, G, c, tid, head_mask, rc_shift, rel_mask, q_shift, bkt, rec, pp.cur, mid);
			} else {
				zero_seen = l1_positions<WIDE_D, C, SLds, REG && FULL, K17, true, true>(L, G, c, tid, head_mask, rc_shift, rel_mask, q_shift, bkt, rec, pp.cur, mid);
			}
			pp.copy_rest((uint32_t)C, slow);
			if (zero_seen) l1_key0_from_chunk(c, head_mask, rc_shift, G.kf, ctr);
			if constexpr (!REG) {
				r0 += stride_r;
				c0 += stride_c;
				if (c0 >= U.Q) { c0 -= U.Q; r0 += 1u; }
			}
			const RawU nxt = fetch(tile + gridDim.x, r0, c0);
			lds_barrier();
			pp.template tail<C, (REG && FULL)>(rec, bkt, zero_seen, [&](uint32_t hist_next) { open_tile(nxt, hist_next); });
			raw = nxt;
		}
		pp.copy_rest(0u, 0ull);
		return;
	}
	if constexpr (LIN && K17 && DBG == 0) {
		const uint32_t tid = fresh_tid();
		const uint32_t sub = blockIdx.x % G.n_sub;
		uint64_t *const out = P.l1 + (uint64_t)sub * G.cap1;
		uint32_t *const cnt = P.cnt1 + sub;
		uint32_t total_prev = 0u;
		static_assert(SLds::kBpt == 1, "thread b owns bucket b");
		auto copy_elem = [&](uint32_t u, uint32_t &slow) {
			const uint32_t p = u * kL1Threads + tid;
			if (p >= total_prev) return;
			const uint64_t rcd = L.stage[p];
			const uint32_t b = L.bucket_of[p];
			const uint64_t off = (uint64_t)(uint32_t)(L.desc[b] + p);
			if (off < G.cap1) out[(uint64_t)b * G.n_sub * G.cap1 + off] = rcd;
			else slow |= 1u << u;
		};
		auto copy_slow = [&](uint32_t slow) {
			for (; slow; slow &= slow - 1u) {
				const uint32_t p = (uint32_t)__builtin_ctz(slow) * kL1Threads + tid;
				const uint64_t rcd = L.stage[p];
				push_overflow(P, record_key(rcd, L.bucket_of[p], G), (uint32_t)(rcd >> 3) & 7u, (uint32_t)rcd & 7u, ctr);
			}
		};
		if (blockIdx.x < n_tiles) {
			open_tile(raw);
			if (tid < 64u) L.hist[kL1MaxB + tid] = 0u;
			lds_barrier();
		}
		for (uint64_t tile = blockIdx.x; tile < n_tiles; tile += gridDim.x) {
			uint32_t word_runs = 0u;
			const Chunk16 c = decode(raw, &word_runs);
			uint32_t bkt[16];
			uint64_t rec[16];
			uint32_t slow = 0u;
			auto mid = [&](uint32_t i) { copy_elem(i, slow); };
			bool zero_seen;
			if constexpr (kRec32) {
				zero_seen = l1_positions<WIDE_D, C, SLds, false, true, true, true>(L, G, c, tid, head_mask, rc_shift, rel_mask, q_shift, bkt, rec, 0u, mid);
			} else {
				if (l1_no_zero_key(k, word_runs))
					zero_seen = l1_positions<WIDE_D, C, SLds, false, true, true, false>(L, G, c, tid, head_mask, rc_shift, rel_mask, q_shift, bkt, rec, 0u, mid);
				else
					zero_seen = l1_positions<WIDE_D, C, SLds, false, true, true, true>(L, G, c, tid, head_mask, rc_shift, rel_mask, q_shift, bkt, rec, 0u, mid);
			}
			if (slow) copy_slow(slow);
			if (zero_seen) l1_key0_from_chunk(c, head_mask, rc_shift, G.kf, ctr);
			r0 += stride_r;
			c0 += stride_c;
			if (c0 >= U.Q) { c0 -= U.Q; r0 += 1u; }
			const RawU nxt = fetch(tile + gridDim.x, r0, c0);
			lds_barrier();
			const uint32_t c_t = L.hist[tid];
			L.hist[tid] = 0u;
			if (tid < 64u) L.hist[kL1MaxB + tid] = 0u;
			const uint32_t g_t = (tid < G.n1 && c_t) ? atomicAdd(&cnt[tid * G.n_sub], c_t) : 0u;
			uint32_t inc = c_t;
			{
				const uint32_t lane = tid & 63u;
#pragma unroll
				for (int off = 1; off < 64; off <<= 1) {
					const uint32_t n = __shfl_up(inc, off, 64);
					if ((int)lane >= off) inc += n;
				}
				if (lane == 63u) L.wave_tot[tid >> 6] = inc;
			}
			lds_barrier();
			uint32_t run = inc - c_t, all = 0;
#pragma unroll
			for (uint32_t w = 0; w < (uint32_t)kL1Threads / 64u; w++) {
				const uint32_t wt = L.wave_tot[w];
				run += (w < (tid >> 6)) ? wt : 0u;
				all += wt;
			}
			L.lbase[tid] = run;
			lds_barrier();
#pragma unroll
			for (int u = 0; u < C; u++) {
				const uint32_t b = bkt[u] >> 16;
				if (b < (uint32_t)kL1MaxB) {
					const uint32_t at = L.lbase[b] + (bkt[u] & 0xFFFFu);
					L.stage[at] = rec[u];
					L.bucket_of[at] = (uint16_t)b;
				}
			}
			L.desc[tid] = g_t - run;
			open_tile(nxt);
			lds_barrier();
			total_prev = all;
			raw = nxt;
		}
		{
			uint32_t slow = 0u;
#pragma unroll 1
			for (uint32_t u = 0; u < (uint32_t)C; u++) copy_elem(u, slow);
			if (slow) copy_slow(slow);
		}
		return;
	}
	for (uint64_t tile = blockIdx.x; tile < n_tiles; tile += gridDim.x) {
		const uint32_t tid = fresh_tid();
		uint32_t bkt[16];
		open_tile(raw);
		lds_barrier();
		const Chunk16 c = decode(raw);
		const bool zero_seen = l1_positions<WIDE_D, C, SLds, REG>(L, G, c, tid, head_mask, rc_shift, rel_mask, q_shift, bkt);
		if (zero_seen) l1_key0_from_chunk(c, head_mask, rc_shift, G.kf, ctr);
		r0 += stride_r;
		c0 += stride_c;
		if (c0 >= U.Q) { c0 -= U.Q; r0 += 1u; }
		if (DBG == 1) {
			uint64_t xx = 0;
#pragma unroll
			for (int u = 0; u < 16; u++) xx ^= L.stage[u * kL1Threads + tid] + bkt[u];
			if (xx == 0x1234567u) P.l1[threadIdx.x] = xx;
			lds_barrier();
			raw = fetch(tile + gridDim.x, r0, c0);
			continue;
		}
		const RawU nxt = fetch(tile + gridDim.x, r0, c0);
		if constexpr (LIN) l1_scatter_tail_linear<DBG, C, (WIDE_D >= 2)>(L, G, P, ctr, tid, bkt);
		else l1_scatter_tail<DBG, (WIDE_D >= 2), (REG ? C : 0)>(L, G, P, ctr, tid, bkt, REG && !zero_seen);
		raw = nxt;
	}
}

struct ReadLanes {
	uint64_t start;
	uint32_t lane0;
	uint32_t W;
};
struct PrefixTile {
	uint64_t B0;
	uint64_t base0;
	uint32_t n_words;
	uint32_t e0;
	uint32_t cc0;
	uint32_t pad;
};
struct PrefixTotals {
	unsigned long long n_lanes, n_entries;
};
constexpr int kPrefixBlock = 1024, kPrefixItems = 4;
constexpr uint32_t kPrefixMaxW = (1u << 22) - 2u;

__device__ __forceinline__ uint32_t prefix_windows(const uint64_t *__restrict__ offsets, uint64_t r, uint32_t k, uint32_t max_read_len)
{
	const uint64_t len = offsets[r + 1] - offsets[r], rl = len > max_read_len ? max_read_len : len;
	return rl >= k ? (uint32_t)(rl - k + 1u) : 0u;
}

template <int C>
__global__ __launch_bounds__(kPrefixBlock) void k_prefix_count(const uint64_t *__restrict__ offsets, uint64_t n_reads, uint32_t k, uint32_t max_read_len,
                                                               unsigned long long *__restrict__ bsum)
{
	__shared__ unsigned long long red[kPrefixBlock / 64];
	const uint64_t first = ((uint64_t)blockIdx.x * kPrefixBlock + threadIdx.x) * kPrefixItems;
	unsigned long long v = 0;
#pragma unroll
	for (int j = 0; j < kPrefixItems; j++)
		if (first + j < n_reads) {
			const uint32_t W = prefix_windows(offsets, first + j, k, max_read_len), Q = (W + (uint32_t)C - 1u) / (uint32_t)C;
			v += (unsigned long long)Q | ((unsigned long long)(Q ? 1u : 0u) << 32);
		}
	const unsigned long long s = block_sum_n<kPrefixBlock>(v, red);
	if (threadIdx.x == 0) bsum[blockIdx.x] = s;
}

__global__ __launch_bounds__(kPrefixBlock) void k_prefix_blocks(unsigned long long *__restrict__ bsum, uint32_t n_blocks, PrefixTotals *__restrict__ tot)
{
	__shared__ unsigned long long wave_tot[kPrefixBlock / 64];
	__shared__ unsigned long long carry;
	const int t = (int)threadIdx.x, lane = t & 63, wave = t >> 6;
	if (t == 0) carry = 0ull;
	__syncthreads();
	for (uint32_t base = 0; base < n_blocks; base += kPrefixBlock) {
		const uint32_t i = base + (uint32_t)t;
		const unsigned long long v = i < n_blocks ? bsum[i] : 0ull;
		unsigned long long inc = v;
#pragma unroll
		for (int off = 1; off < 64; off <<= 1) {
			const unsigned long long n = __shfl_up(inc, off, 64);
			if (lane >= off) inc += n;
		}
		if (lane == 63) wave_tot[wave] = inc;
		__syncthreads();
		unsigned long long before = carry;
		for (int w = 0; w < wave; w++) before += wave_tot[w];
		if (i < n_blocks) bsum[i] = before + inc - v;
		__syncthreads();
		if (t == kPrefixBlock - 1) carry = before + inc;
		__syncthreads();
	}
	if (t == 0) {
		tot->n_lanes = carry & 0xFFFFFFFFull;
		tot->n_entries = carry >> 32;
	}
}

template <int C>
__global__ __launch_bounds__(kPrefixBlock) void k_prefix_emit(const uint64_t *__restrict__ offsets, uint64_t n_reads, uint32_t k, uint32_t max_read_len,
                                                              const unsigned long long *__restrict__ bsum, ReadLanes *__restrict__ ent,
                                                              uint32_t *__restrict__ tile_first, Counters *__restrict__ ctr)
{
	__shared__ unsigned long long wave_tot[kPrefixBlock / 64];
	const int t = (int)threadIdx.x, lane = t & 63, wave = t >> 6;
	const uint64_t first = ((uint64_t)blockIdx.x * kPrefixBlock + threadIdx.x) * kPrefixItems;
	uint32_t W[kPrefixItems];
	unsigned long long v = 0;
#pragma unroll
	for (int j = 0; j < kPrefixItems; j++) {
		W[j] = first + j < n_reads ? prefix_windows(offsets, first + j, k, max_read_len) : 0u;
		const uint32_t Q = (W[j] + (uint32_t)C - 1u) / (uint32_t)C;
		v += (unsigned long long)Q | ((unsigned long long)(Q ? 1u : 0u) << 32);
	}
	unsigned long long inc = v;
#pragma unroll
	for (int off = 1; off < 64; off <<= 1) {
		const unsigned long long n = __shfl_up(inc, off, 64);
		if (lane >= off) inc += n;
	}
	if (lane == 63) wave_tot[wave] = inc;
	__syncthreads();
	unsigned long long run = bsum[blockIdx.x] + inc - v;
	for (int w = 0; w < wave; w++) run += wave_tot[w];
	bool too_long = false;
#pragma unroll
	for (int j = 0; j < kPrefixItems; j++) {
		const uint32_t Q = (W[j] + (uint32_t)C - 1u) / (uint32_t)C;
		if (Q) {
			const uint32_t lane0 = (uint32_t)run, e = (uint32_t)(run >> 32);
			ent[e] = ReadLanes{offsets[first + j], lane0, W[j]};
			too_long = too_long || W[j] > kPrefixMaxW;
			for (uint32_t T = (lane0 + (uint32_t)kL1Threads - 1u) / (uint32_t)kL1Threads; (uint64_t)T * kL1Threads < (uint64_t)lane0 + Q; T++) tile_first[T] = e;
			run += (unsigned long long)Q | (1ull << 32);
		}
	}
	if (too_long) atomicOr(&ctr->error, 4u);
}

template <int C>
__global__ __launch_bounds__(256) void k_prefix_tiles(const ReadLanes *__restrict__ ent, const uint32_t *__restrict__ tile_first,
                                                      const PrefixTotals *__restrict__ tot, uint32_t k, uint64_t n_bases, PrefixTile *__restrict__ tiles)
{
	const uint64_t n_lanes = tot->n_lanes, n_entries = tot->n_entries;
	const uint64_t n_tiles = (n_lanes + kL1Threads - 1) / kL1Threads;
	const uint64_t T = (uint64_t)blockIdx.x * 256 + threadIdx.x;
	if (T >= n_tiles) return;
	const uint32_t e0 = tile_first[T];
	const ReadLanes E0 = ent[e0];
	const uint64_t lane_first = T * kL1Threads, lane_last = min((T + 1) * (uint64_t)kL1Threads, n_lanes) - 1u;
	uint32_t e1 = (uint32_t)n_entries - 1u;
	if (T + 1 < n_tiles) {
		e1 = tile_first[T + 1];
		if ((uint64_t)ent[e1].lane0 > lane_last) e1--;
	}
	const ReadLanes E1 = ent[e1];
	const uint32_t cc0 = (uint32_t)(lane_first - E0.lane0);
	const uint64_t p_first = E0.start + (uint64_t)C * cc0;
	PrefixTile M;
	M.B0 = (p_first ? p_first - 1u : 0u) & ~15ull;
	M.base0 = E0.start;
	uint64_t end = E1.start + (uint64_t)C * (uint32_t)(lane_last - E1.lane0) + (uint32_t)C + k + 2u;
	end = min(end, (n_bases + 15u) & ~15ull);
	const uint64_t words = end > M.B0 ? (end - M.B0 + 15u) >> 4 : 0u;
	M.n_words = (words <= (uint64_t)kPkWords - 8u && E1.start - E0.start < (1ull << 32)) ? (uint32_t)words : 0u;
	M.e0 = e0;
	M.cc0 = cc0;
	M.pad = 0u;
	tiles[T] = M;
}

struct PrefixLds {
	ScatterLds s;
	uint32_t pk[kPkWords];
	uint32_t ent_start[kL1Threads];
	uint32_t meta[kL1Threads];
	unsigned long long starts[2][kL1Threads / 64];
};
static_assert(sizeof(PrefixLds) <= 160 * 1024, "one workgroup per CU");
constexpr uint32_t kPrefixPipeMaxB = (uint32_t)(sizeof(ScatterLds::desc) / 4u) - (uint32_t)(kL1MaxB + 64);

template <int WIDE_D = 0, int C = 16, bool K17 = false>
__global__ __launch_bounds__(kL1Threads) void k_extract_scatter_prefix(ReadBatch rb, const ReadLanes *__restrict__ ent, const PrefixTile *__restrict__ tiles,
                                                                        const PrefixTotals *__restrict__ tot, PartGeom G, PartStore P, Counters *__restrict__ ctr)
{
	extern __shared__ __align__(16) unsigned char lds_raw[];
	PrefixLds &UL = *reinterpret_cast<PrefixLds *>(lds_raw);
	ScatterLds &L = UL.s;
	const uint64_t n_lanes = tot->n_lanes, n_entries = tot->n_entries;
	const uint64_t n_tiles = (n_lanes + kL1Threads - 1) / kL1Threads;
	const uint64_t n_words_total = (rb.n_bases + 15u) >> 4;
	const uint32_t k = (uint32_t)rb.k;
	const uint64_t head_mask = (k < 32u) ? ((1ull << (2u * k)) - 1ull) : ~0ull;
	const uint32_t rc_shift = 2u * k - 2u;
	const uint32_t rel_mask = (1u << G.r) - 1u, q_shift = G.r + 6u;

	struct RawP {
		uint32_t a, b;
		uint32_t start_rel;
		uint32_t meta;
	};
	auto tile_meta = [&](uint64_t tile) {
		PrefixTile M{};
		if (tile < n_tiles) M = tiles[tile];
		return M;
	};
	auto fetch = [&](uint64_t tile, const PrefixTile &M) {
		RawP raw;
		raw.a = raw.b = raw.start_rel = 0u;
		raw.meta = 0xFFFFFFFFu;
		if (tile >= n_tiles) return raw;
		const uint32_t t = fresh_tid();
		const uint64_t w0 = M.B0 >> 4;
		if (t < M.n_words && w0 + t < n_words_total) raw.a = rb.packed[w0 + t];
		if (t + kL1Threads < M.n_words && w0 + t + kL1Threads < n_words_total) raw.b = rb.packed[w0 + t + kL1Threads];
		if ((uint64_t)M.e0 + t < n_entries) {
			const ReadLanes E = ent[(uint64_t)M.e0 + t];
			const uint64_t lane_first = tile * kL1Threads, lane_end = min(lane_first + (uint64_t)kL1Threads, n_lanes);
			if ((uint64_t)E.lane0 < lane_end) {
				const uint32_t at = (uint64_t)E.lane0 > lane_first ? (uint32_t)(E.lane0 - lane_first) : 0u;
				raw.start_rel = (uint32_t)(E.start - M.base0);
				raw.meta = (E.W << 10) | at;
			}
		}
		return raw;
	};
	auto open = [&](const RawP &rw, const PrefixTile &Mx, uint32_t sb, uint32_t hist_off) {
		const uint32_t tid = fresh_tid();
		if (tid < Mx.n_words) UL.pk[tid] = rw.a;
		if (tid + kL1Threads < Mx.n_words) UL.pk[tid + kL1Threads] = rw.b;
		if (rw.meta != 0xFFFFFFFFu) {
			const uint32_t at = rw.meta & 1023u;
			atomicOr(&UL.starts[sb][at >> 6], 1ull << (at & 63u));
			UL.ent_start[tid] = rw.start_rel;
			UL.meta[tid] = rw.meta;
		}
#pragma unroll
		for (int j = 0; j < ScatterLds::kBpt; j++) L.hist[hist_off + ScatterLds::kBpt * tid + j] = 0;
	};
	auto decode = [&](uint64_t tile, const PrefixTile &Mx, uint32_t sb, uint32_t *word_runs = nullptr) {
		const uint32_t tid = fresh_tid();
		const uint64_t lane_first = tile * kL1Threads, lane_end = min(lane_first + (uint64_t)kL1Threads, n_lanes);
		const bool live = lane_first + tid < lane_end;
		uint32_t idx;
		{
			const uint32_t lane = tid & 63u, wave = tid >> 6;
			const unsigned long long mine = UL.starts[sb][wave];
			uint32_t before = (lane < (uint32_t)(kL1Threads / 64) && lane < wave) ? (uint32_t)__popcll(UL.starts[sb][lane]) : 0u;
#pragma unroll
			for (int off = 8; off > 0; off >>= 1) before += __shfl_xor(before, off, 64);
			before = __builtin_amdgcn_readfirstlane(before);
			idx = before + (uint32_t)__popcll(mine & ((2ull << lane) - 1ull)) - 1u;
		}
		uint64_t p = 0;
		uint32_t cc = 0, W = 0;
		if (live) {
			const uint32_t meta = UL.meta[idx];
			W = meta >> 10;
			cc = tid - (meta & 1023u) + (idx == 0u ? Mx.cc0 : 0u);
			p = Mx.base0 + UL.ent_start[idx] + (uint64_t)C * cc;
		}
		const bool no_prev = p == 0u;
		const uint64_t s0 = no_prev ? p : p - 1u;
		const uint32_t first_w = (uint32_t)C * cc;
		Chunk16 c;
		uint32_t x0, x1, x2, x3, x4;
		const uint32_t sh = 2u * ((uint32_t)s0 & 15u);
		if (Mx.n_words) {
			const uint32_t rel = live ? (uint32_t)(s0 - Mx.B0) : 0u;
			const uint32_t d = min(rel >> 4, (uint32_t)kPkWords - 5u);
			x0 = UL.pk[d]; x1 = UL.pk[d + 1]; x2 = UL.pk[d + 2]; x3 = UL.pk[d + 3]; x4 = UL.pk[d + 4];
		} else {
			const uint64_t wi = live ? s0 >> 4 : 0ull, last = n_words_total ? n_words_total - 1u : 0u;
			x0 = rb.packed[min(wi, last)]; x1 = rb.packed[min(wi + 1u, last)]; x2 = rb.packed[min(wi + 2u, last)];
			x3 = rb.packed[min(wi + 3u, last)]; x4 = rb.packed[min(wi + 4u, last)];
		}
		if (word_runs) *word_runs = l1_word_runs(x0, x1, x2, x3, x4);
		const uint32_t X0 = funnel_left(x0, x1, sh), X1 = funnel_left(x1, x2, sh), X2 = funnel_left(x2, x3, sh), X3 = funnel_left(x3, x4, sh);
		const uint32_t adv = no_prev ? 0u : 2u;
		const uint32_t Y0 = funnel_left(X0, X1, adv), Y1 = funnel_left(X1, X2, adv), Y2 = funnel_left(X2, X3, adv), Y3 = X3 << adv;
		c.lw = no_prev ? (X0 >> 2) : X0;
		c.kbit = ((((uint64_t)Y0 << 32) | Y1)) >> (64u - 2u * k);
		c.rc = revcomp_kbit(c.kbit, (int)k);
		const uint32_t widx = k >> 4, wsh = 2u * (k & 15u);
		const uint32_t ya = widx == 0u ? Y0 : (widx == 1u ? Y1 : Y2), yb = widx == 0u ? Y1 : (widx == 1u ? Y2 : Y3);
		c.nb = funnel_left(ya, yb, wsh);
		const uint32_t nv = (live && first_w < W) ? min((uint32_t)C, W - first_w) : 0u;
		const uint32_t nr = (live && first_w + 1u < W) ? min((uint32_t)C, W - 1u - first_w) : 0u;
		c.valid = (1u << nv) - 1u;
		c.has_r = (1u << nr) - 1u;
		c.has_l = cc ? 0xFFFFu : 0xFFFEu;
		return c;
	};

	if (fresh_tid() < (uint32_t)(kL1Threads / 64)) UL.starts[0][fresh_tid()] = UL.starts[1][fresh_tid()] = 0ull;
	PrefixTile M = tile_meta(blockIdx.x), M_next = tile_meta((uint64_t)blockIdx.x + gridDim.x);
	RawP raw = fetch(blockIdx.x, M);
	lds_barrier();
	if constexpr (K17) {
		L1Pipe<false> pp(L, reinterpret_cast<uint32_t *>(L.desc) + (kL1MaxB + 64), G, P, ctr);
		const uint32_t tid = pp.tid;
		uint32_t sb = 0u;
		if (blockIdx.x < n_tiles) {
			open(raw, M, 0u, 0u);
			lds_barrier();
		}
		for (uint64_t tile = blockIdx.x; tile < n_tiles; tile += gridDim.x) {
			uint32_t word_runs = 0u;
			const Chunk16 c = decode(tile, M, sb, &word_runs);
			uint32_t bkt[16];
			uint64_t rec[16];
			uint64_t slow = 0ull;
			auto mid = [&](uint32_t i) { pp.copy_run(i, slow); };
			bool zero_seen;
			if constexpr (WIDE_D == 3) {
				zero_seen = l1_positions<WIDE_D, C, ScatterLds, false, true, true, true>(L, G, c, tid, head_mask, rc_shift, rel_mask, q_shift, bkt, rec, pp.cur, mid);
			} else {
				if (l1_no_zero_key(k, word_runs))
					zero_seen = l1_positions<WIDE_D, C, ScatterLds, false, true, true, false>(L, G, c, tid, head_mask, rc_shift, rel_mask, q_shift, bkt, rec, pp.cur, mid);
				else
					zero_seen = l1_positions<WIDE_D, C, ScatterLds, false, true, true, true>(L, G, c, tid, head_mask, rc_shift, rel_mask, q_shift, bkt, rec, pp.cur, mid);
			}
			pp.copy_rest((uint32_t)C, slow);
			if (zero_seen) l1_key0_from_chunk(c, head_mask, rc_shift, G.kf, ctr);
			const uint64_t t1 = tile + gridDim.x, t2 = t1 + gridDim.x;
			const RawP nxt = fetch(t1, M_next);
			const PrefixTile M_after = tile_meta(t2);
			lds_barrier();
			pp.template tail<C, false>(rec, bkt, zero_seen, [&](uint32_t hist_next) {
				if (tid < (uint32_t)(kL1Threads / 64)) UL.starts[sb][tid] = 0ull;
				open(nxt, M_next, sb ^ 1u, hist_next);
			});
			sb ^= 1u;
			raw = nxt;
			M = M_next;
			M_next = M_after;
		}
		pp.copy_rest(0u, 0ull);
		return;
	}
	for (uint64_t tile = blockIdx.x; tile < n_tiles; tile += gridDim.x) {
		const uint32_t tid = fresh_tid();
		open(raw, M, 0u, 0u);
		uint32_t bkt[16];
		lds_barrier();
		const Chunk16 c = decode(tile, M, 0u);
		const bool zero_seen = l1_positions<WIDE_D, C, ScatterLds, false, K17>(L, G, c, tid, head_mask, rc_shift, rel_mask, q_shift, bkt);
		if (zero_seen) l1_key0_from_chunk(c, head_mask, rc_shift, G.kf, ctr);
		const uint64_t t1 = tile + gridDim.x, t2 = t1 + gridDim.x;
		const RawP nxt = fetch(t1, M_next);
		const PrefixTile M_after = tile_meta(t2);
		lds_barrier();
		if (tid < (uint32_t)(kL1Threads / 64)) UL.starts[0][tid] = 0ull;
		{
			uint64_t rec[16];
#pragma unroll
			for (int u = 0; u < 16; u++) rec[u] = L.stage[u * kL1Threads + tid];
			uint32_t my_gbase[ScatterLds::kBpt];
			const uint32_t sub = blockIdx.x % G.n_sub;
			scatter_reserve_scan(L, G.n1, P.cnt1 + sub, my_gbase, G.n_sub);
			scatter_stage_copy<16, 0, false, (WIDE_D >= 2)>(L, rec, bkt, my_gbase, G.n1, P.l1 + (uint64_t)sub * G.cap1, G.cap1, 0u, true, G, P, ctr, G.n_sub);
		}
		raw = nxt;
		M = M_next;
		M_next = M_after;
	}
}

}
```

Baseline: 108,800.

## Give pipelined L1 scatter its own LDS layout with byte-address bucket words

Introduces dedicated LDS layouts (L1PipeLds, UniformPipeLds, PrefixPipeLds) for the pipelined level-1 scatter. Bucket words now pack the histogram entry's LDS byte address and a byte-scaled rank, so the scatter computes staged addresses with fewer index multiplies and lookups. The scan writes absolute stage byte offsets into lbase. The intent is to cut LDS address arithmetic and free the descriptor array that previously hosted the second histogram, at the cost of a more intricate address encoding and tighter LDS-size assumptions.

```diff
diff --git a/dbg_assembly_amd/csrc/dbgk_host_level1.h b/dbg_assembly_amd/csrc/dbgk_host_level1.h
--- a/dbg_assembly_amd/csrc/dbgk_host_level1.h
+++ b/dbg_assembly_amd/csrc/dbgk_host_level1.h
@@ -11,12 +11,17 @@
 	Fn fn;
 	uint32_t lds;
 };
-template <int DBG, int WIDE_D, int C, bool RAGGED, bool LIN, bool... REST>
-constexpr uint32_t uniform_lds() { return LIN ? sizeof(UniformLdsLin<LIN ? C : 8>) : sizeof(UniformLds); }
+template <int DBG, int WIDE_D, int C, bool RAGGED, bool LIN, bool REG, bool PACKED, bool FULL, bool K17>
+constexpr uint32_t uniform_lds()
+{
+	return LIN ? sizeof(UniformLdsLin<LIN ? C : 8>) : uniform_pipelined(DBG, WIDE_D, RAGGED, LIN, REG, K17) ? sizeof(UniformPipeLds) : sizeof(UniformLds);
+}
+template <int WIDE_D, int C, bool K17>
+constexpr uint32_t prefix_lds() { return K17 ? sizeof(PrefixPipeLds) : sizeof(PrefixLds); }
 #define DBGK_ROW(...) {l1_uniform(__VA_ARGS__), &k_extract_scatter_uniform<__VA_ARGS__>, uniform_lds<__VA_ARGS__>()},
 static const L1Row<decltype(&k_extract_scatter_uniform<>)> kL1UniformRows[] = {DBGK_L1_UNIFORM_ROWS(DBGK_ROW)};
 #undef DBGK_ROW
-#define DBGK_ROW(...) {l1_prefix(__VA_ARGS__), &k_extract_scatter_prefix<__VA_ARGS__>, sizeof(PrefixLds)},
+#define DBGK_ROW(...) {l1_prefix(__VA_ARGS__), &k_extract_scatter_prefix<__VA_ARGS__>, prefix_lds<__VA_ARGS__>()},
 static const L1Row<decltype(&k_extract_scatter_prefix<>)> kL1PrefixRows[] = {DBGK_L1_PREFIX_ROWS(DBGK_ROW)};
 #undef DBGK_ROW
 #define DBGK_ROW(...) {l1_flat(__VA_ARGS__), &k_extract_scatter<__VA_ARGS__>, sizeof(ScatterLds)},
@@ -141,6 +146,10 @@
 		int rc = DBGK_ERR_ARG;
 		switch (l.form.family) {
 		case L1Family::Uniform: {
+			if (g.n_lanes >> 32) {
+				g_last_error = "level 1: a launch of 2^32 lanes or more";
+				return DBGK_ERR_ARG;
+			}
 			ReadBatch r = rb;
 			if (l.n_reads != n_reads) {
 				if (r.packed) r.packed += l.first_read * g.L / 16;
diff --git a/dbg_assembly_amd/csrc/dbgk_partition.h b/dbg_assembly_amd/csrc/dbgk_partition.h
--- a/dbg_assembly_amd/csrc/dbgk_partition.h
+++ b/dbg_assembly_amd/csrc/dbgk_partition.h
@@ -208,9 +208,11 @@
 }
 
 template <class LDS>
-__device__ __forceinline__ void scan_hist_per_wave(LDS &L, uint32_t n_buckets, uint32_t hist_off = 0u)
+__device__ __forceinline__ void scan_hist_per_wave(LDS &L, uint32_t n_buckets, uint32_t hist_off = 0u,
+                                                   uint32_t lbase_off = 0u, uint32_t first = 0u)
 {
 	const uint32_t *hist = L.hist + hist_off;
+	uint32_t *lbase = L.lbase + lbase_off;
 	const uint32_t lane = fresh_tid() & 63u;
 	const uint32_t E = (n_buckets + 63u) >> 6;
 	uint32_t sum = 0;
@@ -224,12 +226,12 @@
 		const uint32_t n = __shfl_up(inc, off, 64);
 		if ((int)lane >= off) inc += n;
 	}
-	uint32_t run = inc - sum;
+	uint32_t run = inc - sum + first;
 	for (uint32_t j = 0; j < E; j++) {
 		const uint32_t b = E * lane + j;
 		if (b < (uint32_t)LDS::kMaxB) {
 			const uint32_t c = hist[b];
-			L.lbase[b] = run;
+			lbase[b] = run;
 			run += c;
 		}
 	}
@@ -248,15 +250,43 @@
 
 constexpr uint32_t kScanStraightB = 256;
 template <class LDS>
-__device__ __forceinline__ void scan_hist_per_wave_256(LDS &L, uint32_t hist_off = 0u)
+__device__ __forceinline__ void scan_hist_per_wave_256(LDS &L, uint32_t hist_off = 0u, uint32_t lbase_off = 0u, uint32_t first = 0u)
 {
 	static_assert(LDS::kMaxB >= (int)kScanStraightB && offsetof(LDS, hist) % 16 == 0 && offsetof(LDS, lbase) % 16 == 0, "16-byte LDS accesses of whole entries");
 	const uint32_t lane = fresh_tid() & 63u;
+	hist_off &= ~3u;
+	lbase_off &= ~3u;
 	const uint4 v = *reinterpret_cast<const uint4 *>(L.hist + hist_off + 4u * lane);
 	const uint32_t sum = (v.x + v.y) + (v.z + v.w);
-	const uint32_t run = wave_scan_inclusive_dpp(sum) - sum;
-	*reinterpret_cast<uint4 *>(L.lbase + 4u * lane) = make_uint4(run, run + v.x, run + v.x + v.y, run + v.x + v.y + v.z);
-}
+	const uint32_t run = wave_scan_inclusive_dpp(sum) - sum + first;
+	*reinterpret_cast<uint4 *>(L.lbase + lbase_off + 4u * lane) = make_uint4(run, run + v.x, run + v.x + v.y, run + v.x + v.y + v.z);
+}
+
+constexpr uint32_t kL1HistWords = (uint32_t)kL1MaxB + 64u;
+constexpr uint32_t kL1RankBits = 17;
+static_assert(8u * (16u * (uint32_t)kL1Threads - 1u) < (1u << kL1RankBits) && 2u * kL1HistWords * 4u <= (1u << (32u - kL1RankBits)), "the two fields of the bucket word");
+__host__ __device__ __forceinline__ uint32_t l1_bucket_word_pack(uint32_t entry_off, uint32_t rank_bytes)
+{
+	return (entry_off << kL1RankBits) | rank_bytes;
+}
+__host__ __device__ __forceinline__ void l1_bucket_word_unpack(uint32_t word, uint32_t &entry_off, uint32_t &rank_bytes)
+{
+	entry_off = word >> kL1RankBits;
+	rank_bytes = word & ((1u << kL1RankBits) - 1u);
+}
+struct L1PipeLds {
+	static constexpr int kThreads = kL1Threads;
+	static constexpr int kRecords = kL1Threads * 16;
+	static constexpr int kMaxB = kL1MaxB;
+	static constexpr int kBpt = kL1MaxB / kL1Threads;
+	uint32_t hist[2 * kL1HistWords];
+	uint32_t lbase[kL1HistWords + kL1MaxB];
+};
+constexpr uint32_t kL1LbaseDist = 2u * kL1HistWords * 4u;
+__device__ __forceinline__ uint32_t lds_address(const void *p) { return (uint32_t)(uintptr_t)(__attribute__((address_space(3))) const void *)p; }
+template <class T>
+__device__ __forceinline__ T *lds_ptr(uint32_t address) { return (T *)(__attribute__((address_space(3))) T *)(uintptr_t)address; }
+static_assert(offsetof(L1PipeLds, hist) == 0 && offsetof(L1PipeLds, lbase) == kL1LbaseDist && sizeof(L1PipeLds) % 16 == 0, "L1PipeLds");
 
 
 template <class LDS>
diff --git a/dbg_assembly_amd/csrc/dbgk_partition_l1.h b/dbg_assembly_amd/csrc/dbgk_partition_l1.h
--- a/dbg_assembly_amd/csrc/dbgk_partition_l1.h
+++ b/dbg_assembly_amd/csrc/dbgk_partition_l1.h
@@ -4,20 +4,23 @@
 
 struct NoMid { __device__ __forceinline__ void operator()(uint32_t) const {} };
 template <int WIDE_D, int NPOS = 16, class LDS = ScatterLds, bool SPECIAL = false, bool ROLL32 = SPECIAL, bool IN_REGS = false, bool ZERO_POSSIBLE = true,
-          class Mid = NoMid>
+          int RANK_BYTES = 0, class Mid = NoMid>
 __device__ __forceinline__ bool l1_positions(LDS &L, const PartGeom &G, Chunk16 c, uint32_t tid, uint64_t head_mask, uint32_t rc_shift,
                                              uint32_t rel_mask, uint32_t q_shift, uint32_t (&bkt)[16], uint64_t *rec = nullptr,
                                              uint32_t hist_off = 0u, Mid mid = Mid())
 {
 	static_assert(!IN_REGS || SPECIAL || ROLL32 || WIDE_D == 3, "records in registers: regular tiles of a graph handle, or a KFREQ handle with direct blocks (nothing to patch)");
 	static_assert(ZERO_POSSIBLE || ((SPECIAL || ROLL32) && WIDE_D != 3), "the positions without the zero-key test: the 32-bit-roll forms of a graph handle");
-	uint32_t *const hh = L.hist + (IN_REGS ? hist_off : 0u);
+	static_assert(RANK_BYTES == 0 || (IN_REGS && (RANK_BYTES == 8 || (RANK_BYTES == 4 && WIDE_D == 3))),
+	              "ranks in bytes: the pipelined tile loop, by the size of the records its L1Pipe stages (4: only a KFREQ handle with direct blocks has 32-bit records)");
+	[[maybe_unused]] uint32_t *const hh = L.hist + ((IN_REGS && !RANK_BYTES) ? hist_off : 0u);
 	const uint32_t lwc = ~c.lw, nbc = ~c.nb;
 	uint32_t rev_mask = 0;
 	bool zero_any = false;
 	uint32_t zero_acc = 0u;
 #pragma unroll
-	for (uint32_t i = NPOS; i < 16; i++) bkt[i] = (uint32_t)kL1MaxB << 16;
+	for (uint32_t i = NPOS; i < 16; i++)
+		bkt[i] = RANK_BYTES ? l1_bucket_word_pack(hist_off + (uint32_t)kL1MaxB * 4u, 0u) : (uint32_t)kL1MaxB << 16;
 #pragma unroll
 	for (uint32_t i = 0; i < (uint32_t)NPOS; i++) {
 		mid(i);
@@ -89,7 +92,12 @@
 			zero_any = zero_any || zero;
 		}
 		const uint32_t b = (valid && !zero) ? bucket : (uint32_t)kL1MaxB + (tid & 63u);
-		bkt[i] = (b << 16) | atomicAdd(&hh[b], 1u);
+		if constexpr (RANK_BYTES != 0) {
+			const uint32_t entry = (b << 2) + hist_off;
+			bkt[i] = l1_bucket_word_pack(entry, atomicAdd(lds_ptr<uint32_t>(entry), (uint32_t)RANK_BYTES));
+		} else {
+			bkt[i] = (b << 16) | atomicAdd(&hh[b], 1u);
+		}
 		if constexpr (ROLL32) {
 			const uint32_t klo = (uint32_t)c.kbit, khi = (uint32_t)(c.kbit >> 32);
 			const uint32_t nhi = __builtin_amdgcn_alignbit(khi, klo, 30u) & (uint32_t)(head_mask >> 32), nlo = (klo << 2) | right;
@@ -131,17 +139,18 @@
 			}
 		}
 		return zero_acc != 0u;
-	}
-	for (uint32_t fix = (WIDE_D == 3 || (!SPECIAL && G.kf)) ? 0u : ((no_l | no_r) & c.valid); fix; fix &= fix - 1u) {
-		const uint32_t i = (uint32_t)__builtin_ctz(fix);
-		const bool fwd = !((rev_mask >> ((uint32_t)NPOS - 1u - i)) & 1u), nl = (no_l >> i) & 1u, nr = (no_r >> i) & 1u;
-		uint64_t rec = L.stage[i * kL1Threads + tid];
-		uint32_t lb = ((uint32_t)rec >> 3) & 7u, rbb = (uint32_t)rec & 7u;
-		if (fwd ? nl : nr) lb = 4u;
-		if (fwd ? nr : nl) rbb = 4u;
-		L.stage[i * kL1Threads + tid] = (rec & ~63ull) | (lb << 3) | rbb;
-	}
-	return zero_any;
+	} else {
+		for (uint32_t fix = (WIDE_D == 3 || (!SPECIAL && G.kf)) ? 0u : ((no_l | no_r) & c.valid); fix; fix &= fix - 1u) {
+			const uint32_t i = (uint32_t)__builtin_ctz(fix);
+			const bool fwd = !((rev_mask >> ((uint32_t)NPOS - 1u - i)) & 1u), nl = (no_l >> i) & 1u, nr = (no_r >> i) & 1u;
+			uint64_t rec = L.stage[i * kL1Threads + tid];
+			uint32_t lb = ((uint32_t)rec >> 3) & 7u, rbb = (uint32_t)rec & 7u;
+			if (fwd ? nl : nr) lb = 4u;
+			if (fwd ? nr : nl) rbb = 4u;
+			L.stage[i * kL1Threads + tid] = (rec & ~63ull) | (lb << 3) | rbb;
+		}
+		return zero_any;
+	}
 }
 
 template <int DBG, bool KF32_POSSIBLE = true, int N_SURE = 0>
@@ -344,8 +353,18 @@
 struct UniformLds {
 	ScatterLds s;
 	uint32_t pk[kPkWords];
-	uint32_t gbase[kL1MaxB];
 };
+struct UniformPipeLds {
+	uint32_t pk[kPkWords];
+	L1PipeLds s;
+	uint64_t stage[L1PipeLds::kRecords];
+};
+static_assert(offsetof(UniformPipeLds, stage) <= 64 * 1024 && offsetof(UniformPipeLds, stage) % 16 == 0 && sizeof(UniformPipeLds) <= 160 * 1024, "one workgroup per CU");
+static_assert(offsetof(UniformPipeLds, s) % 16 == 0 && offsetof(UniformPipeLds, s) + sizeof(L1PipeLds::hist) <= (1u << (32u - kL1RankBits)), "a histogram entry's LDS address is a field of the bucket word");
+constexpr bool uniform_pipelined(int dbg, int wide_d, bool ragged, bool lin, bool reg, bool k17)
+{
+	return !lin && dbg == 0 && (reg || k17 || (wide_d == 3 && !ragged));
+}
 template <int C>
 struct UniformLdsLin {
 	ScatterLdsLin<C> s;
@@ -386,15 +405,16 @@
 	}
 }
 
-template <bool REC32>
+template <bool REC32, uint32_t STAGE_OFF>
 struct L1Pipe {
 	static constexpr uint32_t kWaves = kL1Threads / 64;
-	static constexpr uint32_t kHist2 = (uint32_t)((offsetof(ScatterLds, desc) - offsetof(ScatterLds, hist)) / 4u);
-	static_assert(sizeof(ScatterLds::desc) >= sizeof(ScatterLds::hist), "the second histogram lives in the descriptor array");
+	static constexpr uint32_t kHist2 = kL1HistWords;
+	static constexpr uint32_t kRecShift = REC32 ? 2u : 3u;
 	static_assert(kL1MaxB <= kL1Threads, "thread b reserves bucket b");
 	static_assert(kHist2 % 4u == 0u, "scan_hist_per_wave_256 reads either histogram sixteen bytes at a time");
-	ScatterLds &L;
-	uint32_t *const gbase;
+	static_assert(STAGE_OFF % 16u == 0u && STAGE_OFF >= sizeof(L1PipeLds) && 160u * 1024u / 4u < (1u << 16),
+	              "a run's first staged record, in records from LDS address 0, travels in sixteen bits of d_lo");
+	L1PipeLds &L;
 	const PartGeom &G;
 	const PartStore &P;
 	Counters *const ctr;
@@ -402,11 +422,18 @@
 	uint64_t *out;
 	uint32_t *cnt;
 	uint64_t bucket_stride;
+	uint32_t cap32;
 	uint32_t d_lo = 0u, d_gb = 0u;
 	uint32_t cur = 0u;
 
-	__device__ __forceinline__ L1Pipe(ScatterLds &L_, uint32_t *gbase_, const PartGeom &G_, const PartStore &P_, Counters *ctr_)
-	    : L(L_), gbase(gbase_), G(G_), P(P_), ctr(ctr_)
+	__device__ __forceinline__ uint32_t lds0() const { return lds_address(&L); }
+	__device__ __forceinline__ uint32_t cur_at() const
+	{
+		uint32_t at = lds0() + (uint32_t)offsetof(L1PipeLds, hist) + 4u * cur;
+		asm volatile("" : "+s"(at));
+		return at;
+	}
+	__device__ __forceinline__ L1Pipe(L1PipeLds &L_, const PartGeom &G_, const PartStore &P_, Counters *ctr_) : L(L_), G(G_), P(P_), ctr(ctr_)
 	{
 		tid = fresh_tid();
 		lane = tid & 63u;
@@ -417,33 +444,38 @@
 		out = P.l1 + (uint64_t)sub * G.cap1;
 		cnt = P.cnt1 + sub;
 		bucket_stride = (uint64_t)G.n_sub * G.cap1;
-	}
-	__device__ __forceinline__ uint32_t *stage32() const { return reinterpret_cast<uint32_t *>(L.stage); }
+		cap32 = __builtin_amdgcn_readfirstlane((uint32_t)(G.cap1 >> 32) ? 0xFFFFFFFFu : (uint32_t)G.cap1);
+	}
+	__device__ __forceinline__ uint64_t staged64(uint32_t i) const { return *lds_ptr<const uint64_t>(8u * i); }
+	__device__ __forceinline__ uint32_t staged32(uint32_t i) const { return *lds_ptr<const uint32_t>(4u * i); }
 
 	__device__ __forceinline__ void copy_run(uint32_t kk, uint64_t &slow) const
 	{
 		const uint32_t lo = __builtin_amdgcn_readlane(d_lo, kk), dst = __builtin_amdgcn_readlane(d_gb, kk);
 		const uint32_t n = lo >> 16, src = lo & 0xFFFFu;
 		if (n == 0u) return;
-		if ((uint64_t)dst + n > G.cap1) {
+		const uint64_t end = (uint64_t)dst + n;
+		uint32_t end_hi = (uint32_t)(end >> 32);
+		asm volatile("" : "+s"(end_hi));
+		if (end_hi != 0u || (uint32_t)end > cap32) {
 			slow |= 1ull << kk;
 			return;
 		}
-		uint32_t b = wave + kWaves * kk;
-		asm volatile("" : "+s"(b));
+		uint32_t w = wave;
+		asm volatile("" : "+s"(w));
+		const uint32_t b = w + kWaves * kk;
 		if constexpr (REC32) {
 			static_assert(kSubStores == 1, "the 32-bit level-1 store is addressed without sub-stores");
 			uint32_t *o32 = reinterpret_cast<uint32_t *>(out) + (uint64_t)b * G.cap1 + dst;
-			const uint32_t *s32 = stage32();
 			typedef uint32_t u32x4_a4 __attribute__((ext_vector_type(4), aligned(4)));
 			if (n >= 4u) {
 				for (uint32_t i = 4u * lane; i < n; i += 256u) {
 					const uint32_t j = min(i, n - 4u);
-					const u32x4_a4 v = {s32[src + j], s32[src + j + 1u], s32[src + j + 2u], s32[src + j + 3u]};
+					const u32x4_a4 v = {staged32(src + j), staged32(src + j + 1u), staged32(src + j + 2u), staged32(src + j + 3u)};
 					*reinterpret_cast<u32x4_a4 *>(o32 + j) = v;
 				}
 			} else if (lane < n) {
-				o32[lane] = s32[src + lane];
+				o32[lane] = staged32(src + lane);
 			}
 			return;
 		}
@@ -452,12 +484,12 @@
 		if (n >= 2u) {
 			for (uint32_t i = 2u * lane; i < n; i += 128u) {
 				const uint32_t j = min(i, n - 2u);
-				const uint64_t a = L.stage[src + j], b2 = L.stage[src + j + 1u];
+				const uint64_t a = staged64(src + j), b2 = staged64(src + j + 1u);
 				const u32x4_a8 v = {(uint32_t)a, (uint32_t)(a >> 32), (uint32_t)b2, (uint32_t)(b2 >> 32)};
 				*reinterpret_cast<u32x4_a8 *>(o + j) = v;
 			}
 		} else if (lane == 0u) {
-			o[0] = L.stage[src];
+			o[0] = staged64(src);
 		}
 	}
 	__device__ __forceinline__ void copy_slow(uint64_t slow) const
@@ -470,7 +502,7 @@
 			uint64_t *o = out + (uint64_t)b * G.n_sub * G.cap1 + dst;
 			uint32_t *o32 = reinterpret_cast<uint32_t *>(out) + (uint64_t)b * G.cap1 + dst;
 			for (uint32_t i = lane; i < n; i += 64u) {
-				const uint64_t rcd = REC32 ? (uint64_t)stage32()[src + i] : L.stage[src + i];
+				const uint64_t rcd = REC32 ? (uint64_t)staged32(src + i) : staged64(src + i);
 				if ((uint64_t)dst + i < G.cap1) {
 					if constexpr (REC32) o32[i] = (uint32_t)rcd;
 					else o[i] = rcd;
@@ -486,30 +518,41 @@
 	template <int C, bool SURE, class Open>
 	__device__ __forceinline__ void tail(const uint64_t (&rec)[16], const uint32_t (&bkt)[16], bool zero_seen, Open open_next)
 	{
-		const uint32_t c_t = tid < G.n1 ? L.hist[cur + tid] : 0u;
+		uint32_t n1 = G.n1;
+		asm volatile("" : "+s"(n1));
+		const uint32_t c_t = tid < n1 ? L.hist[cur + tid] >> kRecShift : 0u;
 		const uint32_t g_t = c_t ? atomicAdd(&cnt[tid * G.n_sub], c_t) : 0u;
 		const uint32_t c_mine = lane < per_wave ? L.hist[cur + mine] : 0u;
-		if (G.n1 <= kScanStraightB) scan_hist_per_wave_256(L, cur);
-		else scan_hist_per_wave(L, G.n1, cur);
-		d_lo = (c_mine << 16) | (lane < per_wave ? L.lbase[mine] : 0u);
+		if (n1 <= kScanStraightB) scan_hist_per_wave_256(L, cur, cur, lds0() + STAGE_OFF);
+		else scan_hist_per_wave(L, n1, cur, cur, lds0() + STAGE_OFF);
+		d_lo = (c_mine << (16u - kRecShift)) | (lane < per_wave ? L.lbase[cur + mine] >> kRecShift : 0u);
+		auto first_of = [&](uint32_t word) {
+			uint32_t entry, rank;
+			l1_bucket_word_unpack(word, entry, rank);
+			return *lds_ptr<const uint32_t>(entry + kL1LbaseDist);
+		};
+		auto put = [&](uint32_t first, uint32_t word, uint64_t r) {
+			uint32_t entry, rank;
+			l1_bucket_word_unpack(word, entry, rank);
+			if constexpr (REC32) *lds_ptr<uint32_t>(first + rank) = (uint32_t)r;
+			else *lds_ptr<uint64_t>(first + rank) = r;
+		};
 		if (SURE && __builtin_amdgcn_ballot_w64(zero_seen) == 0ull) {
 			uint32_t at[C];
 #pragma unroll
-			for (int u = 0; u < C; u++) at[u] = L.lbase[bkt[u] >> 16];
-#pragma unroll
-			for (int u = 0; u < C; u++) L.stage[at[u] + (bkt[u] & 0xFFFFu)] = rec[u];
+			for (int u = 0; u < C; u++) at[u] = first_of(bkt[u]);
+#pragma unroll
+			for (int u = 0; u < C; u++) put(at[u], bkt[u], rec[u]);
 		} else {
+			const uint32_t no_bucket = l1_bucket_word_pack(cur_at() + (uint32_t)kL1MaxB * 4u, 0u);
 #pragma unroll
 			for (int u = 0; u < C; u++)
-				if ((bkt[u] >> 16) < (uint32_t)kL1MaxB) {
-					if constexpr (REC32) stage32()[L.lbase[bkt[u] >> 16] + (bkt[u] & 0xFFFFu)] = (uint32_t)rec[u];
-					else L.stage[L.lbase[bkt[u] >> 16] + (bkt[u] & 0xFFFFu)] = rec[u];
-				}
-		}
-		if (tid < G.n1) gbase[tid] = g_t;
+				if (bkt[u] < no_bucket) put(first_of(bkt[u]), bkt[u], rec[u]);
+		}
+		if (tid < n1) L.lbase[(cur ^ kHist2) + tid] = g_t;
 		open_next(cur ^ kHist2);
 		lds_barrier();
-		d_gb = lane < per_wave ? gbase[mine] : 0u;
+		d_gb = lane < per_wave ? L.lbase[(cur ^ kHist2) + mine] : 0u;
 		cur ^= kHist2;
 	}
 };
@@ -524,8 +567,11 @@
 	static_assert(!PACKED || REG, "the other forms test rb.packed at run time");
 	static_assert(FULL || (REG && DBG == 0), "partly filled lanes: the pipelined regular tiles");
 	static_assert(K17 || !REG, "regular tiles: k >= 17");
-	using ULds = typename std::conditional<LIN, UniformLdsLin<LIN ? C : 8>, UniformLds>::type;
-	using SLds = typename std::conditional<LIN, ScatterLdsLin<LIN ? C : 8>, ScatterLds>::type;
+	constexpr bool kRec32 = WIDE_D == 3;
+	constexpr bool kPipe = uniform_pipelined(DBG, WIDE_D, RAGGED, LIN, REG, K17);
+	constexpr bool kZeroPerWave = K17 && !kRec32;
+	using ULds = typename std::conditional<LIN, UniformLdsLin<LIN ? C : 8>, typename std::conditional<kPipe, UniformPipeLds, UniformLds>::type>::type;
+	using SLds = typename std::conditional<LIN, ScatterLdsLin<LIN ? C : 8>, typename std::conditional<kPipe, L1PipeLds, ScatterLds>::type>::type;
 	extern __shared__ __align__(16) unsigned char lds_raw[];
 	ULds &UL = *reinterpret_cast<ULds *>(lds_raw);
 	SLds &L = UL.s;
@@ -557,11 +603,17 @@
 		else raw.a = raw.b = make_uint4(0x41414141u, 0x41414141u, 0x41414141u, 0x41414141u);
 		raw.B0 = raw.p = 0;
 		raw.n_blocks = raw.cc = raw.W = 0;
-		if (tile >= n_tiles) return raw;
+		if constexpr (REG) {
+			if ((uint32_t)tile >= (uint32_t)n_tiles) return raw;
+		} else {
+			if (tile >= n_tiles) return raw;
+		}
 		const uint32_t t = fresh_tid();
 		if constexpr (REG) {
-			raw.B0 = tile * ((uint64_t)U.tile_blocks * 16u);
-			raw.n_blocks = U.tile_blocks;
+			uint32_t tile_blocks = U.tile_blocks;
+			asm volatile("" : "+s"(tile_blocks));
+			raw.B0 = tile * ((uint64_t)tile_blocks * 16u);
+			raw.n_blocks = tile_blocks;
 			if constexpr (PACKED) {
 				const uint32_t *words = rb.packed + (raw.B0 >> 4);
 				if (t < raw.n_blocks) raw.a = words[t];
@@ -621,25 +673,42 @@
 		}
 #pragma unroll
 		for (int j = 0; j < SLds::kBpt; j++) L.hist[hist_off + SLds::kBpt * tid + j] = 0;
+		if constexpr (kPipe) {
+			if (tid < 64u) L.hist[hist_off + (uint32_t)kL1MaxB + tid] = 0;
+		}
 	};
+	uint32_t lane_at = 0u, lane_nsh = 0u, lane_cc = 0u;
+	if constexpr (REG && FULL) {
+		const uint32_t t = fresh_tid();
+		lane_cc = t & (U.Q - 1u);
+		const uint32_t rel = (t >> U.lq) * U.L + (uint32_t)C * lane_cc - (lane_cc == 0u ? 0u : 1u);
+		lane_at = ((rel >> 4) << 2) + lds_address(UL.pk);
+		lane_nsh = 32u - 2u * (rel & 15u);
+	}
 	auto decode = [&](const RawU &raw, uint32_t *word_runs = nullptr) {
 		if constexpr (REG && FULL) {
-			const uint32_t t = fresh_tid();
-			const uint32_t cc = t & (U.Q - 1u);
-			const bool first = cc == 0u, last = cc == U.Q - 1u;
-			const uint32_t rel = (t >> U.lq) * U.L + (uint32_t)C * cc - (first ? 0u : 1u);
-			const uint32_t d = rel >> 4, sh = 2u * (rel & 15u);
-			const uint32_t x0 = UL.pk[d], x1 = UL.pk[d + 1], x2 = UL.pk[d + 2], x3 = UL.pk[d + 3], x4 = UL.pk[d + 4];
+			uint32_t at = lane_at, nsh = lane_nsh, cc = lane_cc;
+			asm volatile("" : "+v"(at), "+v"(nsh), "+v"(cc));
+			uint32_t ks = k;
+			asm volatile("" : "+s"(ks));
+			const bool first = cc == 0u, last = cc == U.Q - 1u, sh0 = nsh == 32u;
+			const uint32_t *const w = lds_ptr<const uint32_t>(at);
+			const uint32_t x0 = w[0], x1 = w[1], x2 = w[2], x3 = w[3], x4 = w[4];
 			if (word_runs) *word_runs = l1_word_runs(x0, x1, x2, x3, x4);
-			const uint32_t X0 = funnel_left(x0, x1, sh), X1 = funnel_left(x1, x2, sh), X2 = funnel_left(x2, x3, sh), X3 = funnel_left(x3, x4, sh);
+			auto funnel = [&](uint32_t hi, uint32_t lo) {
+				uint32_t f = __builtin_amdgcn_alignbit(hi, lo, nsh);
+				asm volatile("" : "+v"(f));
+				return sh0 ? hi : f;
+			};
+			const uint32_t X0 = funnel(x0, x1), X1 = funnel(x1, x2), X2 = funnel(x2, x3), X3 = funnel(x3, x4);
 			const uint32_t adv = first ? 0u : 2u;
 			const uint32_t Y0 = funnel_left(X0, X1, adv), Y1 = funnel_left(X1, X2, adv), Y2 = funnel_left(X2, X3, adv), Y3 = X3 << adv;
 			Chunk16 c;
 			c.lw = first ? (X0 >> 2) : X0;
-			c.kbit = ((((uint64_t)Y0 << 32) | Y1)) >> (64u - 2u * k);
-			c.rc = revcomp_kbit(c.kbit, (int)k);
-			const bool k32 = (k >> 4) == 2u;
-			const uint32_t wsh = 2u * (k & 15u);
+			c.kbit = ((((uint64_t)Y0 << 32) | Y1)) >> (64u - 2u * ks);
+			c.rc = revcomp_kbit(c.kbit, (int)ks);
+			const bool k32 = (ks >> 4) == 2u;
+			const uint32_t wsh = 2u * (ks & 15u);
 			c.nb = funnel_left(k32 ? Y2 : Y1, k32 ? Y3 : Y2, wsh);
 			c.valid = (1u << C) - 1u;
 			c.has_r = last ? (1u << (C - 1)) - 1u : (1u << C) - 1u;
@@ -672,11 +741,9 @@
 		c.has_l = raw.cc ? 0xFFFFu : 0xFFFEu;
 		return c;
 	};
-	constexpr bool kRec32 = WIDE_D == 3;
-	constexpr bool kPipe = !LIN && DBG == 0 && (REG || K17 || (kRec32 && !RAGGED));
-	constexpr bool kZeroPerWave = K17 && !kRec32;
 	if constexpr (kPipe) {
-		L1Pipe<kRec32> pp(L, UL.gbase, G, P, ctr);
+		constexpr int kRB = kRec32 ? 4 : 8;
+		L1Pipe<kRec32, (uint32_t)(offsetof(UniformPipeLds, stage) - offsetof(UniformPipeLds, s))> pp(L, G, P, ctr);
 		const uint32_t tid = pp.tid;
 		if (blockIdx.x < n_tiles) {
 			open_tile(raw, 0u);
@@ -692,11 +759,11 @@
 			bool zero_seen;
 			if constexpr (kZeroPerWave) {
 				if (l1_no_zero_key(k, word_runs))
-					zero_seen = l1_positions<WIDE_D, C, SLds, REG && FULL, K17, true, false>(L, G, c, tid, head_mask, rc_shift, rel_mask, q_shift, bkt, rec, pp.cur, mid);
+					zero_seen = l1_positions<WIDE_D, C, SLds, REG && FULL, K17, true, false, kRB>(L, G, c, tid, head_mask, rc_shift, rel_mask, q_shift, bkt, rec, pp.cur_at(), mid);
 				else
-					zero_seen = l1_positions<WIDE_D, C, SLds, REG && FULL, K17, true, true>(L, G, c, tid, head_mask, rc_shift, rel_mask, q_shift, bkt, rec, pp.cur, mid);
+					zero_seen = l1_positions<WIDE_D, C, SLds, REG && FULL, K17, true, true, kRB>(L, G, c, tid, head_mask, rc_shift, rel_mask, q_shift, bkt, rec, pp.cur_at(), mid);
 			} else {
-				zero_seen = l1_positions<WIDE_D, C, SLds, REG && FULL, K17, true, true>(L, G, c, tid, head_mask, rc_shift, rel_mask, q_shift, bkt, rec, pp.cur, mid);
+				zero_seen = l1_positions<WIDE_D, C, SLds, REG && FULL, K17, true, true, kRB>(L, G, c, tid, head_mask, rc_shift, rel_mask, q_shift, bkt, rec, pp.cur_at(), mid);
 			}
 			pp.copy_rest((uint32_t)C, slow);
 			if (zero_seen) l1_key0_from_chunk(c, head_mask, rc_shift, G.kf, ctr);
@@ -711,9 +778,8 @@
 			raw = nxt;
 		}
 		pp.copy_rest(0u, 0ull);
-		return;
-	}
-	if constexpr (LIN && K17 && DBG == 0) {
+	}
+	else if constexpr (LIN && K17 && DBG == 0) {
 		const uint32_t tid = fresh_tid();
 		const uint32_t sub = blockIdx.x % G.n_sub;
 		uint64_t *const out = P.l1 + (uint64_t)sub * G.cap1;
@@ -809,32 +875,32 @@
 			for (uint32_t u = 0; u < (uint32_t)C; u++) copy_elem(u, slow);
 			if (slow) copy_slow(slow);
 		}
-		return;
-	}
-	for (uint64_t tile = blockIdx.x; tile < n_tiles; tile += gridDim.x) {
-		const uint32_t tid = fresh_tid();
-		uint32_t bkt[16];
-		open_tile(raw);
-		lds_barrier();
-		const Chunk16 c = decode(raw);
-		const bool zero_seen = l1_positions<WIDE_D, C, SLds, REG>(L, G, c, tid, head_mask, rc_shift, rel_mask, q_shift, bkt);
-		if (zero_seen) l1_key0_from_chunk(c, head_mask, rc_shift, G.kf, ctr);
-		r0 += stride_r;
-		c0 += stride_c;
-		if (c0 >= U.Q) { c0 -= U.Q; r0 += 1u; }
-		if (DBG == 1) {
-			uint64_t xx = 0;
-#pragma unroll
-			for (int u = 0; u < 16; u++) xx ^= L.stage[u * kL1Threads + tid] + bkt[u];
-			if (xx == 0x1234567u) P.l1[threadIdx.x] = xx;
-			lds_barrier();
-			raw = fetch(tile + gridDim.x, r0, c0);
-			continue;
-		}
-		const RawU nxt = fetch(tile + gridDim.x, r0, c0);
-		if constexpr (LIN) l1_scatter_tail_linear<DBG, C, (WIDE_D >= 2)>(L, G, P, ctr, tid, bkt);
-		else l1_scatter_tail<DBG, (WIDE_D >= 2), (REG ? C : 0)>(L, G, P, ctr, tid, bkt, REG && !zero_seen);
-		raw = nxt;
+	} else {
+		for (uint64_t tile = blockIdx.x; tile < n_tiles; tile += gridDim.x) {
+			const uint32_t tid = fresh_tid();
+			uint32_t bkt[16];
+			open_tile(raw);
+			lds_barrier();
+			const Chunk16 c = decode(raw);
+			const bool zero_seen = l1_positions<WIDE_D, C, SLds, REG>(L, G, c, tid, head_mask, rc_shift, rel_mask, q_shift, bkt);
+			if (zero_seen) l1_key0_from_chunk(c, head_mask, rc_shift, G.kf, ctr);
+			r0 += stride_r;
+			c0 += stride_c;
+			if (c0 >= U.Q) { c0 -= U.Q; r0 += 1u; }
+			if (DBG == 1) {
+				uint64_t xx = 0;
+#pragma unroll
+				for (int u = 0; u < 16; u++) xx ^= L.stage[u * kL1Threads + tid] + bkt[u];
+				if (xx == 0x1234567u) P.l1[threadIdx.x] = xx;
+				lds_barrier();
+				raw = fetch(tile + gridDim.x, r0, c0);
+				continue;
+			}
+			const RawU nxt = fetch(tile + gridDim.x, r0, c0);
+			if constexpr (LIN) l1_scatter_tail_linear<DBG, C, (WIDE_D >= 2)>(L, G, P, ctr, tid, bkt);
+			else l1_scatter_tail<DBG, (WIDE_D >= 2), (REG ? C : 0)>(L, G, P, ctr, tid, bkt, REG && !zero_seen);
+			raw = nxt;
+		}
 	}
 }
 
@@ -992,15 +1058,28 @@
 	unsigned long long starts[2][kL1Threads / 64];
 };
 static_assert(sizeof(PrefixLds) <= 160 * 1024, "one workgroup per CU");
-constexpr uint32_t kPrefixPipeMaxB = (uint32_t)(sizeof(ScatterLds::desc) / 4u) - (uint32_t)(kL1MaxB + 64);
+struct PrefixPipeLds {
+	uint32_t pk[kPkWords];
+	L1PipeLds s;
+	uint32_t ent_start[kL1Threads];
+	uint32_t meta[kL1Threads];
+	unsigned long long starts[2][kL1Threads / 64];
+	uint64_t stage[L1PipeLds::kRecords];
+};
+static_assert(offsetof(PrefixPipeLds, stage) <= 64 * 1024 && offsetof(PrefixPipeLds, stage) % 16 == 0 && sizeof(PrefixPipeLds) <= 160 * 1024, "one workgroup per CU");
+static_assert(offsetof(PrefixPipeLds, s) == offsetof(UniformPipeLds, s), "the bucket word's entry field");
+constexpr uint32_t kPrefixPipeMaxB = 960;
+static_assert(kPrefixPipeMaxB <= (uint32_t)kL1MaxB, "L1PipeLds holds kL1MaxB buckets");
 
 template <int WIDE_D = 0, int C = 16, bool K17 = false>
 __global__ __launch_bounds__(kL1Threads) void k_extract_scatter_prefix(ReadBatch rb, const ReadLanes *__restrict__ ent, const PrefixTile *__restrict__ tiles,
                                                                         const PrefixTotals *__restrict__ tot, PartGeom G, PartStore P, Counters *__restrict__ ctr)
 {
 	extern __shared__ __align__(16) unsigned char lds_raw[];
-	PrefixLds &UL = *reinterpret_cast<PrefixLds *>(lds_raw);
-	ScatterLds &L = UL.s;
+	using ULds = typename std::conditional<K17, PrefixPipeLds, PrefixLds>::type;
+	using SLds = typename std::conditional<K17, L1PipeLds, ScatterLds>::type;
+	ULds &UL = *reinterpret_cast<ULds *>(lds_raw);
+	SLds &L = UL.s;
 	const uint64_t n_lanes = tot->n_lanes, n_entries = tot->n_entries;
 	const uint64_t n_tiles = (n_lanes + kL1Threads - 1) / kL1Threads;
 	const uint64_t n_words_total = (rb.n_bases + 15u) >> 4;
@@ -1050,7 +1129,10 @@
 			UL.meta[tid] = rw.meta;
 		}
 #pragma unroll
-		for (int j = 0; j < ScatterLds::kBpt; j++) L.hist[hist_off + ScatterLds::kBpt * tid + j] = 0;
+		for (int j = 0; j < SLds::kBpt; j++) L.hist[hist_off + SLds::kBpt * tid + j] = 0;
+		if constexpr (K17) {
+			if (tid < 64u) L.hist[hist_off + (uint32_t)kL1MaxB + tid] = 0;
+		}
 	};
 	auto decode = [&](uint64_t tile, const PrefixTile &Mx, uint32_t sb, uint32_t *word_runs = nullptr) {
 		const uint32_t tid = fresh_tid();
@@ -1112,7 +1194,7 @@
 	RawP raw = fetch(blockIdx.x, M);
 	lds_barrier();
 	if constexpr (K17) {
-		L1Pipe<false> pp(L, reinterpret_cast<uint32_t *>(L.desc) + (kL1MaxB + 64), G, P, ctr);
+		L1Pipe<false, (uint32_t)(offsetof(PrefixPipeLds, stage) - offsetof(PrefixPipeLds, s))> pp(L, G, P, ctr);
 		const uint32_t tid = pp.tid;
 		uint32_t sb = 0u;
 		if (blockIdx.x < n_tiles) {
@@ -1128,12 +1210,12 @@
 			auto mid = [&](uint32_t i) { pp.copy_run(i, slow); };
 			bool zero_seen;
 			if constexpr (WIDE_D == 3) {
-				zero_seen = l1_positions<WIDE_D, C, ScatterLds, false, true, true, true>(L, G, c, tid, head_mask, rc_shift, rel_mask, q_shift, bkt, rec, pp.cur, mid);
+				zero_seen = l1_positions<WIDE_D, C, SLds, false, true, true, true, 8>(L, G, c, tid, head_mask, rc_shift, rel_mask, q_shift, bkt, rec, pp.cur_at(), mid);
 			} else {
 				if (l1_no_zero_key(k, word_runs))
-					zero_seen = l1_positions<WIDE_D, C, ScatterLds, false, true, true, false>(L, G, c, tid, head_mask, rc_shift, rel_mask, q_shift, bkt, rec, pp.cur, mid);
+					zero_seen = l1_positions<WIDE_D, C, SLds, false, true, true, false, 8>(L, G, c, tid, head_mask, rc_shift, rel_mask, q_shift, bkt, rec, pp.cur_at(), mid);
 				else
-					zero_seen = l1_positions<WIDE_D, C, ScatterLds, false, true, true, true>(L, G, c, tid, head_mask, rc_shift, rel_mask, q_shift, bkt, rec, pp.cur, mid);
+					zero_seen = l1_positions<WIDE_D, C, SLds, false, true, true, true, 8>(L, G, c, tid, head_mask, rc_shift, rel_mask, q_shift, bkt, rec, pp.cur_at(), mid);
 			}
 			pp.copy_rest((uint32_t)C, slow);
 			if (zero_seen) l1_key0_from_chunk(c, head_mask, rc_shift, G.kf, ctr);
@@ -1151,34 +1233,34 @@
 			M_next = M_after;
 		}
 		pp.copy_rest(0u, 0ull);
-		return;
-	}
-	for (uint64_t tile = blockIdx.x; tile < n_tiles; tile += gridDim.x) {
-		const uint32_t tid = fresh_tid();
-		open(raw, M, 0u, 0u);
-		uint32_t bkt[16];
-		lds_barrier();
-		const Chunk16 c = decode(tile, M, 0u);
-		const bool zero_seen = l1_positions<WIDE_D, C, ScatterLds, false, K17>(L, G, c, tid, head_mask, rc_shift, rel_mask, q_shift, bkt);
-		if (zero_seen) l1_key0_from_chunk(c, head_mask, rc_shift, G.kf, ctr);
-		const uint64_t t1 = tile + gridDim.x, t2 = t1 + gridDim.x;
-		const RawP nxt = fetch(t1, M_next);
-		const PrefixTile M_after = tile_meta(t2);
-		lds_barrier();
-		if (tid < (uint32_t)(kL1Threads / 64)) UL.starts[0][tid] = 0ull;
-		{
-			uint64_t rec[16];
-#pragma unroll
-			for (int u = 0; u < 16; u++) rec[u] = L.stage[u * kL1Threads + tid];
-			uint32_t my_gbase[ScatterLds::kBpt];
-			const uint32_t sub = blockIdx.x % G.n_sub;
-			scatter_reserve_scan(L, G.n1, P.cnt1 + sub, my_gbase, G.n_sub);
-			scatter_stage_copy<16, 0, false, (WIDE_D >= 2)>(L, rec, bkt, my_gbase, G.n1, P.l1 + (uint64_t)sub * G.cap1, G.cap1, 0u, true, G, P, ctr, G.n_sub);
-		}
-		raw = nxt;
-		M = M_next;
-		M_next = M_after;
-	}
-}
-
-}
+	} else {
+		for (uint64_t tile = blockIdx.x; tile < n_tiles; tile += gridDim.x) {
+			const uint32_t tid = fresh_tid();
+			open(raw, M, 0u, 0u);
+			uint32_t bkt[16];
+			lds_barrier();
+			const Chunk16 c = decode(tile, M, 0u);
+			const bool zero_seen = l1_positions<WIDE_D, C, ScatterLds, false, K17>(L, G, c, tid, head_mask, rc_shift, rel_mask, q_shift, bkt);
+			if (zero_seen) l1_key0_from_chunk(c, head_mask, rc_shift, G.kf, ctr);
+			const uint64_t t1 = tile + gridDim.x, t2 = t1 + gridDim.x;
+			const RawP nxt = fetch(t1, M_next);
+			const PrefixTile M_after = tile_meta(t2);
+			lds_barrier();
+			if (tid < (uint32_t)(kL1Threads / 64)) UL.starts[0][tid] = 0ull;
+			{
+				uint64_t rec[16];
+#pragma unroll
+				for (int u = 0; u < 16; u++) rec[u] = L.stage[u * kL1Threads + tid];
+				uint32_t my_gbase[ScatterLds::kBpt];
+				const uint32_t sub = blockIdx.x % G.n_sub;
+				scatter_reserve_scan(L, G.n1, P.cnt1 + sub, my_gbase, G.n_sub);
+				scatter_stage_copy<16, 0, false, (WIDE_D >= 2)>(L, rec, bkt, my_gbase, G.n1, P.l1 + (uint64_t)sub * G.cap1, G.cap1, 0u, true, G, P, ctr, G.n_sub);
+			}
+			raw = nxt;
+			M = M_next;
+			M_next = M_after;
+		}
+	}
+}
+
+}
```

Result: faster. 110,000 (median of 6 runs) (+1.0%).
